# widdowquinn/pyani

Hardware: AMD Instinct MI355X
Metric: genome-pairs/sec (ordered pairs) + wall-clock for the N x N ANIm grid: nucmer --mum + delta-filter -1 + parse_delta equivalent per ordered pair, genomes resident in HBM; vs the CPU path on this box's host cores (higher is better)
Workload: dtype u32 packed DP words (score << 17 | state << 15 | errors), i64 lengths, f64 identity

## Files before the change

### pyani_amd/csrc/pg_anim.hip

```cpp
#include <tuple>
#include "pg_internal.h"
#include "pg_anim_core.h"
#include "pg_nucmer_core.h"
#include "pg_nucmer_diag.h"
#include "pg_anib_core.h"
#include "pg_anim_trace.h"

using namespace pga;

namespace {

constexpr unsigned long long SLOT_EMPTY = ~0ull;
constexpr int FRAG_SEED_MIN = 16;

struct RefDesc {
  const uint32_t* codes;
  const uint32_t* mask;
  int32_t len;
  const int32_t* rec_start;
  int32_t n_rec;
};

struct UnitDesc {
  const uint32_t* codes;
  const uint32_t* mask;
  int32_t len;
  const int32_t* rec_start;
  int32_t n_rec;
  int32_t strand;
  int32_t pair;
  int32_t ref;
};

__device__ __forceinline__ void get16(const uint32_t* __restrict__ codes, const uint32_t* __restrict__ mask, int32_t p,
                                      uint32_t& c, uint32_t& m) {
  const uint32_t cw = p >> 4, cs = 2 * (p & 15);
  const uint64_t lo = (uint64_t)codes[cw] | ((uint64_t)codes[cw + 1] << 32);
  c = (uint32_t)(lo >> cs);
  const uint32_t mw = p >> 5, ms = p & 31;
  const uint64_t ml = (uint64_t)mask[mw] | ((uint64_t)mask[mw + 1] << 32);
  m = (uint32_t)(ml >> ms) & 0xFFFFu;
}

__device__ __forceinline__ void packed_window(const uint32_t* __restrict__ codes, const uint32_t* __restrict__ mask, int32_t len, int64_t p0,
                                              uint64_t& c, uint32_t& ok) {
  c = 0; ok = 0;
  if (p0 >= len || p0 + 32 <= 0) return;
  const int64_t q0 = p0 < 0 ? 0 : p0;
  const int sh = (int)(q0 - p0);
  const int32_t w = (int32_t)(q0 >> 4), lastw = (len - 1) >> 4;
  const uint32_t c0 = codes[w], c1 = codes[w + 1 <= lastw ? w + 1 : lastw], c2 = codes[w + 2 <= lastw ? w + 2 : lastw];
  const int cs = 2 * (int)(q0 & 15);
  uint64_t lo = ((uint64_t)c1 << 32) | c0;
  uint64_t win = cs ? ((lo >> cs) | ((uint64_t)c2 << (64 - cs))) : lo;
  const int32_t mw = (int32_t)(q0 >> 5), lastm = (len - 1) >> 5;
  const uint64_t m = ((uint64_t)mask[mw + 1 <= lastm ? mw + 1 : lastm] << 32) | mask[mw];
  uint32_t okw = (uint32_t)(m >> (q0 & 31));
  const int64_t avail = len - q0;
  if (avail < 32) okw &= (avail <= 0 ? 0u : ((1u << avail) - 1u));
  c = sh ? (win << (2 * sh)) : win;
  ok = sh ? (okw << sh) : okw;
}

#include "pga_seed.inc"
#include "pga_cluster.inc"
#include "pga_postnuc.inc"
#include "pga_finish.inc"
#include "pga_frag.inc"

}

namespace {
struct GenomeIdx {
  uint64_t *ref_list = nullptr, *qry_list = nullptr, *qry_list1 = nullptr;
  uint32_t *ref_goff = nullptr, *qry_goff = nullptr, *qry_goff1 = nullptr;
  uint32_t ref_max = 0;
  uint32_t* word_start = nullptr;
  int32_t* word_pos = nullptr;
};
struct AnimLists { std::vector<GenomeIdx> gidx; };
thread_local PgAlnSink* tls_sink = nullptr;
thread_local int tls_worker = 0;

struct AnimScratch {
  size_t units = 0, pairs = 0, refs = 0, recs = 0, wl = 0, matches = 0;
  uint32_t* list_cnt = nullptr;
  SeedRef* srefs_d = nullptr;
  SeedQry* sqry_d = nullptr;
  SeedSlice* slice_d = nullptr;
  size_t slice_pairs = 0;
  int32_t* recs_d = nullptr;
  RefDesc* refs_d = nullptr;
  UnitDesc* units_d = nullptr;
  uint32_t *mem_count = nullptr, *moff = nullptr, *choff_d = nullptr;
  int32_t *nch = nullptr, *status = nullptr;
  pg_anim_result* out = nullptr;
  Match *mem = nullptr, *cm = nullptr;
  int32_t *iscratch = nullptr, *order = nullptr;
  Chain* chains = nullptr;
  FinishScratch S{};
  uint2* wl_d = nullptr;
  Match* seedbuf = nullptr;
  size_t seed_cap = 0;
  uint32_t* seed_total = nullptr;
  Match* hits_d = nullptr;
  Match* hits_sorted = nullptr;
  uint32_t *hit_count = nullptr, *hoff = nullptr, *hit_cursor = nullptr;
  size_t hit_cap = 0;
  int32_t* mirror_d = nullptr;
  BigUnit* big_d = nullptr;
  uint2* ranges_d = nullptr;
  RangeOut* range_out = nullptr;
  size_t big_cap = 0, range_cap = 0;
  bool lds_attr_set = false;
  pgn::PnAln* pn = nullptr;
  uint8_t* pn_fused = nullptr;
  int32_t* pn_n = nullptr;
  uint32_t* pn_cursor = nullptr;
  uint32_t* pn_gscratch = nullptr;
  uint32_t* pn_wide = nullptr;
  PnForcedReq* pn_reqs = nullptr;
  pgn::PnGap* pn_gaps = nullptr;
  pgn::PnFwd* pn_fwd = nullptr;
  pgn::PnBwd* pn_bwd = nullptr;
  pgn::PnTurn* pn_tlog = nullptr;
  int32_t* pn_born = nullptr;
  uint32_t* pn_porder = nullptr;
  pgn::PnPiece* pn_pieces = nullptr;
  uint32_t* pn_npieces = nullptr;
  size_t pn_piece_cap = 0, pn_npieces_cap = 0;
  uint8_t* tr_arena = nullptr;
  uint32_t* tr_out = nullptr;
  PnTraceJob* tr_jobs = nullptr;
  unsigned long long *tr_off = nullptr, *tr_cursor = nullptr;
  int32_t* tr_cnt = nullptr;
  size_t tr_arena_cap = 0, tr_out_cap = 0, tr_jobs_cap = 0;
  PnGapTask* pn_tasks = nullptr;
  uint32_t* pn_order = nullptr;
  size_t pn_cap = 0, pn_units = 0, pn_waves = 0, pn_req_cap = 0, pn_req_n = 0;
  int32_t* fr_tables = nullptr;
  FragPair* fr_pairs = nullptr;
  uint32_t *fr_slot_pair = nullptr, *fr_off = nullptr, *fr_nrows = nullptr;
  uint64_t* fr_ebase = nullptr;
  FragSeed* fr_entries = nullptr;
  FragRow* fr_rows = nullptr;
  pg_anib_result* fr_out = nullptr;
  uint32_t *fr_list = nullptr, *fr_nlist = nullptr, *fr_wtmp = nullptr;
  WordIdx* fr_widx = nullptr;
  size_t fr_list_cap = 0, fr_widx_cap = 0;
  size_t fr_tables_cap = 0, fr_pairs_cap = 0, fr_slots_cap = 0, fr_off_cap = 0, fr_units_cap = 0, fr_entries_cap = 0;
};

template <typename T>
int regrow(pg_ctx* ctx, T*& p, size_t n) {
  if (p) PG_HIP(ctx, hipFree(p));
  p = nullptr;
  PG_HIP(ctx, hipMalloc(reinterpret_cast<void**>(&p), (n ? n : 1) * sizeof(T)));
  return PG_OK;
}
}

static AnimScratch* anim_scratch(pg_ctx* ctx) {
  void*& slot = tls_worker ? ctx->anim_scratch_w[tls_worker] : ctx->anim_scratch;
  if (!slot) slot = new AnimScratch();
  return static_cast<AnimScratch*>(slot);
}
static AnimLists* anim_lists(pg_ctx* ctx) {
  if (!ctx->anim_lists) ctx->anim_lists = new AnimLists();
  return static_cast<AnimLists*>(ctx->anim_lists);
}
static hipStream_t cur_stream(pg_ctx* ctx) { return tls_worker ? ctx->stream_w[tls_worker] : ctx->stream; }
void pg_anim_set_worker(pg_ctx* ctx, int worker) {
  tls_worker = worker > 0 && worker < pg_ctx::MAX_WORKERS ? worker : 0;
  pg_tls_stream = cur_stream(ctx);
}

void pg_anim_set_sink(PgAlnSink* sink) { tls_sink = sink; }
int pg_anim_counters_read(pg_ctx* ctx, uint64_t* out, int reset) {
  PG_HIP(ctx, hipDeviceSynchronize());
  unsigned long long a[32], b[32], z[32] = {0};
  PG_HIP(ctx, hipMemcpyFromSymbol(a, HIP_SYMBOL(g_pn_stats), sizeof(a)));
  PG_HIP(ctx, hipMemcpyFromSymbol(b, HIP_SYMBOL(g_pn_kstats), sizeof(b)));
  for (int i = 0; i < 32; ++i) { out[i] = a[i]; out[32 + i] = b[i]; }
  if (reset) {
    PG_HIP(ctx, hipMemcpyToSymbol(HIP_SYMBOL(g_pn_stats), z, sizeof(z)));
    PG_HIP(ctx, hipMemcpyToSymbol(HIP_SYMBOL(g_pn_kstats), z, sizeof(z)));
  }
  return PG_OK;
}

void pg_anim_drop_lists(pg_ctx* ctx) {
  std::lock_guard<std::mutex> lk(ctx->anim_mu);
  AnimLists* A = static_cast<AnimLists*>(ctx->anim_lists);
  if (!A) return;
  for (auto& g : A->gidx) {
    void* ptrs[] = {g.ref_list, g.qry_list, g.ref_goff, g.qry_goff, g.qry_list1, g.qry_goff1, g.word_start, g.word_pos};
    for (void* p : ptrs) if (p) (void)hipFree(p);
  }
  A->gidx.clear();
}

static int anim_ensure_lists(pg_ctx* ctx, AnimScratch* A, const std::vector<int32_t>& ref_genomes, const std::vector<int32_t>& qry_genomes,
                             int qstep) {
  std::lock_guard<std::mutex> lk(ctx->anim_mu);
  AnimLists* LS = anim_lists(ctx);
  if (LS->gidx.size() < ctx->genomes.size()) LS->gidx.resize(ctx->genomes.size());
  std::vector<std::pair<uint64_t**, uint32_t**>> mine;
  const int rc_all = [&]() -> int {
  int rc;
  bool built = false;
  if (!A->list_cnt && (rc = regrow(ctx, A->list_cnt, (size_t)2 * SEED_GROUPS))) return rc;
  std::vector<int32_t> fresh_refs;
  for (int role = 0; role < 2; ++role) {
    for (int32_t gid : role ? qry_genomes : ref_genomes) {
      GenomeIdx& X = LS->gidx[gid];
      uint64_t*& qlist = qstep == 1 ? X.qry_list1 : X.qry_list;
      uint32_t*& qgoff = qstep == 1 ? X.qry_goff1 : X.qry_goff;
      if (role ? qlist != nullptr : X.ref_list != nullptr) continue;
      const PgGenome& G = ctx->genomes[gid];
      const int32_t len = (int32_t)G.stream_len;
      const uint32_t n_sub = role ? 2 * SEED_GROUPS : SEED_GROUPS;
      const size_t bound = role ? 2 * ((size_t)len / qstep + 1) : (size_t)len + 1;
      uint64_t*& list = role ? qlist : X.ref_list;
      uint32_t*& goff = role ? qgoff : X.ref_goff;
      mine.emplace_back(&list, &goff);
      if ((rc = regrow(ctx, list, bound))) return rc;
      if ((rc = regrow(ctx, goff, (size_t)n_sub + 2))) return rc;
      const uint32_t* codes = ctx->d_codes + G.arena_start / 16;
      const uint32_t* mask = ctx->d_mask + G.arena_start / 32;
      const int32_t n_idx = role ? len / qstep + 1 : len;
      const dim3 grid((uint32_t)(n_idx + LIST_CHUNK - 1) / LIST_CHUNK, role ? 2 : 1);
      PG_HIP(ctx, hipMemsetAsync(A->list_cnt, 0, (size_t)n_sub * 4, cur_stream(ctx)));
      if (grid.x)
        hipLaunchKernelGGL(anim_list_kernel, grid, dim3(LIST_BLOCK), 0, cur_stream(ctx), codes, mask, len, role, A->list_cnt,
                           (const uint32_t*)nullptr, (uint64_t*)nullptr, 0, qstep);
      hipLaunchKernelGGL(anim_list_scan_kernel, dim3(1), dim3(64), 0, cur_stream(ctx), A->list_cnt, goff, n_sub);
      if (grid.x)
        hipLaunchKernelGGL(anim_list_kernel, grid, dim3(LIST_BLOCK), 0, cur_stream(ctx), codes, mask, len, role, A->list_cnt,
                           (const uint32_t*)goff, list, 1, qstep);
      if (!role) fresh_refs.push_back(gid);
      built = true;
    }
  }
  PG_HIP(ctx, hipGetLastError());
  if (built) PG_HIP(ctx, hipStreamSynchronize(cur_stream(ctx)));
  for (int32_t gid : fresh_refs)
    PG_HIP(ctx, hipMemcpy(&LS->gidx[gid].ref_max, LS->gidx[gid].ref_goff + SEED_GROUPS + 1, 4, hipMemcpyDeviceToHost));
  return PG_OK;
  }();
  if (rc_all != PG_OK) {
    (void)hipStreamSynchronize(cur_stream(ctx));
    for (auto& pr : mine) {
      if (*pr.first) { (void)hipFree(*pr.first); *pr.first = nullptr; }
      if (*pr.second) { (void)hipFree(*pr.second); *pr.second = nullptr; }
    }
  }
  return rc_all;
}

static void anim_free_one(pg_ctx* ctx, void*& slot);
void pg_anim_release_worker_scratch(pg_ctx* ctx) {
  (void)hipStreamSynchronize(ctx->stream);
  for (int w = 1; w < pg_ctx::MAX_WORKERS; ++w) (void)hipStreamSynchronize(ctx->stream_w[w]);
  anim_free_one(ctx, ctx->anim_scratch);
  for (int w = 1; w < pg_ctx::MAX_WORKERS; ++w) anim_free_one(ctx, ctx->anim_scratch_w[w]);
  ctx->anim_scratch_matches_held = 0;
}
void pg_anim_free_scratch(pg_ctx* ctx) {
  pg_anim_drop_lists(ctx);
  delete static_cast<AnimLists*>(ctx->anim_lists);
  ctx->anim_lists = nullptr;
  anim_free_one(ctx, ctx->anim_scratch);
  for (int w = 1; w < pg_ctx::MAX_WORKERS; ++w) anim_free_one(ctx, ctx->anim_scratch_w[w]);
  ctx->anim_scratch_matches_held = 0;
}
static void anim_free_one(pg_ctx* ctx, void*& slot) {
  AnimScratch* A = static_cast<AnimScratch*>(slot);
  if (!A) return;
  void* ptrs[] = {A->mirror_d, A->big_d, A->ranges_d, A->range_out, A->hits_sorted, A->hit_count, A->hoff, A->hit_cursor, A->hits_d, A->slice_d, A->choff_d, A->list_cnt, A->srefs_d, A->sqry_d, A->recs_d, A->refs_d, A->units_d, A->mem_count, A->moff, A->nch, A->status, A->out, A->mem, A->cm,
                  A->iscratch, A->order, A->chains, A->S.alns, A->S.a_rrec,
                  A->S.a_qrec, A->S.idx, A->S.from, A->S.sc, A->wl_d, A->seedbuf, A->seed_total, A->fr_tables, A->fr_pairs,
                  A->fr_slot_pair, A->fr_off, A->fr_nrows, A->fr_ebase, A->fr_entries, A->fr_rows, A->fr_out, A->fr_list, A->fr_nlist, A->fr_wtmp, A->fr_widx,
                  A->pn, A->pn_fused, A->pn_n, A->pn_cursor, A->pn_gscratch, A->pn_reqs, A->pn_wide, A->pn_gaps, A->pn_fwd, A->pn_bwd, A->pn_tlog, A->pn_born, A->pn_porder, A->pn_tasks, A->pn_order, A->pn_pieces, A->pn_npieces, A->tr_arena, A->tr_out, A->tr_jobs, A->tr_off, A->tr_cursor, A->tr_cnt};
  for (void* p : ptrs) if (p) (void)hipFree(p);
  delete A;
  slot = nullptr;
}

static_assert(sizeof(FragRow) == sizeof(pg_anib_row), "FragRow is pg_anib_row");
static int anib_frag_stage(pg_ctx* ctx, AnimScratch* A, const int32_t* qry_ids, uint32_t n_pairs, const std::vector<uint32_t>& cnt,
                           const PgFragArgs& F, const std::vector<int32_t>& ref_list, const std::vector<uint32_t>& ref_of_pair);

static int anim_collect(pg_ctx* ctx, AnimScratch* A, const int32_t* ref_ids, const int32_t* qry_ids, uint32_t n_pairs, const pg_anim_result* res,
                        const std::vector<uint32_t>& choff, PgAlnSink& sink) {
  const uint32_t n_units = 2 * n_pairs;
  int rc;
  std::vector<uint32_t> moff((size_t)n_units + 1);
  PG_HIP(ctx, hipMemcpy(moff.data(), A->moff, moff.size() * 4, hipMemcpyDeviceToHost));
  const size_t total = moff[n_units];
  std::vector<Aln> al(total ? total : 1);
  std::vector<int32_t> rr(total ? total : 1), qr(total ? total : 1);
  if (total) {
    PG_HIP(ctx, hipMemcpy(al.data(), A->S.alns, total * sizeof(Aln), hipMemcpyDeviceToHost));
    PG_HIP(ctx, hipMemcpy(rr.data(), A->S.a_rrec, total * 4, hipMemcpyDeviceToHost));
    PG_HIP(ctx, hipMemcpy(qr.data(), A->S.a_qrec, total * 4, hipMemcpyDeviceToHost));
  }
  const size_t first_aln = sink.alns.size();
  std::vector<size_t> pair_first(n_pairs);
  for (uint32_t p = 0; p < n_pairs; ++p) {
    if (res[p].status == PG_E_CAPACITY) return pg_fail(ctx, PG_E_CAPACITY, "anim: work buffers overflowed for a pair of the batch");
    const PgGenome& G = ctx->genomes[ref_ids[p]];
    const PgGenome& H = ctx->genomes[qry_ids[p]];
    const uint32_t n = (uint32_t)res[p].reserved;
    pair_first[p] = sink.alns.size();
    for (uint32_t i = 0; i < n; ++i) {
      const Aln& a = al[moff[2 * p] + i];
      const int32_t r_ = rr[moff[2 * p] + i], q_ = qr[moff[2 * p] + i], ro = G.rec_start[r_], qo = H.rec_start[q_];
      pg_anim_alignment x;
      x.ref_rec = r_; x.qry_rec = q_;
      x.rs = a.rs - ro + 1; x.re = a.re - ro;
      x.qs = a.strand ? a.qe - qo : a.qs - qo + 1;
      x.qe = a.strand ? a.qs - qo + 1 : a.qe - qo;
      x.errors = a.errors; x.kept = a.keep;
      sink.alns.push_back(x);
    }
    sink.pair_count.push_back(n);
  }
  if (!sink.with_indels) return PG_OK;
  sink.indels.resize(sink.alns.size());
  const size_t n_wl = choff[n_units];
  if (!total || !n_wl) return PG_OK;
  std::vector<pgn::PnAln> pn(total);
  std::vector<int32_t> pn_n(n_units);
  std::vector<uint32_t> npieces(n_units);
  const size_t piece_total = pn_piece_base(total, (uint32_t)n_wl, n_units);
  std::vector<pgn::PnPiece> pieces(piece_total ? piece_total : 1);
  PG_HIP(ctx, hipMemcpy(pn.data(), A->pn, total * sizeof(pgn::PnAln), hipMemcpyDeviceToHost));
  PG_HIP(ctx, hipMemcpy(pn_n.data(), A->pn_n, (size_t)n_units * 4, hipMemcpyDeviceToHost));
  PG_HIP(ctx, hipMemcpy(npieces.data(), A->pn_npieces, (size_t)n_units * 4, hipMemcpyDeviceToHost));
  PG_HIP(ctx, hipMemcpy(pieces.data(), A->pn_pieces, piece_total * sizeof(pgn::PnPiece), hipMemcpyDeviceToHost));
  const size_t req_cap = A->pn_req_n;
  std::vector<PnForcedReq> reqs(req_cap);
  PG_HIP(ctx, hipMemcpy(reqs.data(), A->pn_reqs, req_cap * sizeof(PnForcedReq), hipMemcpyDeviceToHost));
  struct JobRef { uint32_t unit; uint32_t piece; uint64_t bytes; };
  std::vector<PnTraceJob> jobs;
  std::vector<JobRef> refs_;
  for (uint32_t u = 0; u < n_units; ++u) {
    const size_t pb = pn_piece_base(moff[u], choff[u], u);
    if (pn_n[u] < 0 || npieces[u] > pn_piece_cap((size_t)moff[u + 1] - moff[u], choff[u + 1] - choff[u]))
      return pg_fail(ctx, PG_E_CAPACITY, "anim traceback: a unit's piece list overflowed");
    for (uint32_t k = 0; k < npieces[u]; ++k) {
      const pgn::PnPiece& P = pieces[pb + k];
      if (P.kind == pgn::PIECE_MATCH || P.kind == pgn::PIECE_VISIT) continue;
      PnTraceJob J{};
      J.unit = u; J.m_o = P.m_o; J.A0 = P.A0; J.B0 = P.B0; J.A1 = P.A1; J.B1 = P.B1;
      uint64_t cells = P.cells;
      uint32_t wmax = P.wmax;
      if (P.kind == pgn::PIECE_FORCED) {
        J.tA = P.A1; J.tB = P.B1;
        if (P.aux >= req_cap) return pg_fail(ctx, PG_E_INTERNAL, "anim traceback: forced piece without its request");
        J.band_w = reqs[P.aux].w;
        const int32_t N = P.A1 - P.A0 + 1, M_ = P.B1 - P.B0 + 1;
        cells = 0; wmax = 0;
        for (int32_t d = 1; d <= N + M_; ++d) {
          int32_t lo = d - N > 0 ? d - N : 0, hi = d < M_ ? d : M_;
          if (J.band_w >= 0) pgn::forced_band_clip(d, N, M_, J.band_w, lo, hi);
          if (hi >= lo) { cells += (uint64_t)(hi - lo + 1); if ((uint32_t)(hi - lo + 1) > wmax) wmax = (uint32_t)(hi - lo + 1); }
        }
      } else {
        J.tA = P.tA; J.tB = P.tB; J.band_w = -1;
        if (P.cells == 0xFFFFFFFFu) return pg_fail(ctx, PG_E_CAPACITY, "anim traceback: a search outgrew the register engine");
      }
      const int32_t N = J.tA - J.A0 + 1, M_ = J.tB - J.B0 + 1;
      J.cap = wmax + 2; J.dcap = (uint32_t)(N + M_ + 4); J.rle_cap = (uint32_t)(N + M_ + 4); J.bp_cap = cells;
      const uint64_t bytes = (uint64_t)J.cap * 3 * sizeof(pgn::Cell) + (uint64_t)J.dcap * 8 + (uint64_t)J.rle_cap * 4 + ((cells + 15) & ~15ull) + 16;
      jobs.push_back(J);
      refs_.push_back(JobRef{u, k, (bytes + 15) & ~15ull});
    }
  }
  std::vector<uint32_t> order(jobs.size());
  for (uint32_t i = 0; i < order.size(); ++i) order[i] = i;
  std::stable_sort(order.begin(), order.end(), [&](uint32_t a, uint32_t b) { return refs_[a].bytes > refs_[b].bytes; });
  std::vector<std::vector<uint32_t>> rle(jobs.size());
  const uint64_t ARENA = 6ull << 30, OUT_MAX = 192ull << 20;
  if (!A->tr_cursor && (rc = regrow(ctx, A->tr_cursor, 2))) return rc;
  for (size_t b0 = 0; b0 < order.size();) {
    uint64_t bytes = 0, outs = 0;
    size_t b1 = b0;
    while (b1 < order.size() && (b1 == b0 || (bytes + refs_[order[b1]].bytes <= ARENA && outs + jobs[order[b1]].rle_cap <= OUT_MAX))) {
      bytes += refs_[order[b1]].bytes; outs += jobs[order[b1]].rle_cap; ++b1;
    }
    const size_t nb = b1 - b0;
    std::vector<PnTraceJob> hj(nb);
    uint64_t at = 0;
    for (size_t k = 0; k < nb; ++k) { hj[k] = jobs[order[b0 + k]]; hj[k].slab = at; at += refs_[order[b0 + k]].bytes; }
    if (bytes > A->tr_arena_cap) { if ((rc = regrow(ctx, A->tr_arena, (size_t)bytes))) return rc; A->tr_arena_cap = (size_t)bytes; }
    if (outs > A->tr_out_cap) { if ((rc = regrow(ctx, A->tr_out, (size_t)outs))) return rc; A->tr_out_cap = (size_t)outs; }
    if (nb > A->tr_jobs_cap) {
      if ((rc = regrow(ctx, A->tr_jobs, nb))) return rc;
      if ((rc = regrow(ctx, A->tr_off, nb))) return rc;
      if ((rc = regrow(ctx, A->tr_cnt, nb))) return rc;
      A->tr_jobs_cap = nb;
    }
    PG_HIP(ctx, hipMemcpyAsync(A->tr_jobs, hj.data(), nb * sizeof(PnTraceJob), hipMemcpyHostToDevice, cur_stream(ctx)));
    PG_HIP(ctx, hipMemsetAsync(A->tr_cursor, 0, 8, cur_stream(ctx)));
    hipLaunchKernelGGL(anim_trace_kernel, dim3((uint32_t)((nb + 63) / 64)), dim3(64), 0, cur_stream(ctx), A->refs_d, A->units_d, A->tr_jobs, (uint32_t)nb,
                       A->tr_arena, A->tr_out, (unsigned long long)outs, A->tr_cursor, A->tr_off, A->tr_cnt);
    PG_HIP(ctx, hipGetLastError());
    std::vector<unsigned long long> off(nb);
    std::vector<int32_t> cnt(nb);
    unsigned long long used = 0;
    PG_HIP(ctx, hipMemcpyAsync(off.data(), A->tr_off, nb * 8, hipMemcpyDeviceToHost, cur_stream(ctx)));
    PG_HIP(ctx, hipMemcpyAsync(cnt.data(), A->tr_cnt, nb * 4, hipMemcpyDeviceToHost, cur_stream(ctx)));
    PG_HIP(ctx, hipMemcpyAsync(&used, A->tr_cursor, 8, hipMemcpyDeviceToHost, cur_stream(ctx)));
    PG_HIP(ctx, hipStreamSynchronize(cur_stream(ctx)));
    std::vector<uint32_t> out((size_t)used ? (size_t)used : 1);
    if (used) PG_HIP(ctx, hipMemcpy(out.data(), A->tr_out, (size_t)used * 4, hipMemcpyDeviceToHost));
    for (size_t k = 0; k < nb; ++k) {
      if (cnt[k] < 0) return pg_fail(ctx, PG_E_INTERNAL, "anim traceback: a piece did not repeat in the scalar engine");
      rle[order[b0 + k]].assign(out.begin() + (size_t)off[k], out.begin() + (size_t)off[k] + (size_t)cnt[k]);
    }
    b0 = b1;
  }
  size_t job_at = 0;
  for (uint32_t p = 0; p < n_pairs; ++p) {
    const size_t n_rec = (size_t)pn_n[2 * p] + (size_t)pn_n[2 * p + 1];
    if (n_rec != sink.pair_count[sink.pair_count.size() - n_pairs + p]) return pg_fail(ctx, PG_E_INTERNAL, "anim traceback: record counts differ");
    std::vector<std::vector<int64_t>> lists(n_rec);
    std::vector<std::tuple<int32_t, int32_t, int32_t>> key(n_rec);
    for (uint32_t u = 2 * p; u < 2 * p + 2; ++u) {
      const size_t pb = pn_piece_base(moff[u], choff[u], u);
      std::vector<int32_t> job_of(npieces[u], -1);
      for (uint32_t k = 0; k < npieces[u]; ++k)
        if (pieces[pb + k].kind == pgn::PIECE_SEARCH || pieces[pb + k].kind == pgn::PIECE_FORCED) job_of[k] = (int32_t)job_at++;
      std::vector<std::vector<int64_t>> deltas;
      std::vector<int32_t> visit;
      std::string why;
      static const uint32_t none = 0;
      if (!pgt::unit_deltas(pieces.data() + pb, (int32_t)npieces[u], pn.data() + moff[u], pn_n[u],
                            [&](int32_t k, int32_t& c) -> const uint32_t* { const auto& v = rle[(size_t)job_of[k]]; c = (int32_t)v.size(); return v.empty() ? &none : v.data(); },
                            deltas, visit, &why))
        return pg_fail(ctx, PG_E_INTERNAL, "anim traceback: " + why);
      const size_t base = (u & 1) ? (size_t)pn_n[u - 1] : 0;
      for (int32_t i = 0; i < pn_n[u]; ++i) { lists[base + (size_t)i] = std::move(deltas[(size_t)i]); key[base + (size_t)i] = std::make_tuple(visit[(size_t)i], (int32_t)(u & 1), i); }
    }
    std::vector<size_t> perm(n_rec);
    for (size_t i = 0; i < n_rec; ++i) perm[i] = i;
    std::stable_sort(perm.begin(), perm.end(), [&](size_t a, size_t b) { return key[a] < key[b]; });
    std::vector<pg_anim_alignment> recs(n_rec);
    for (size_t i = 0; i < n_rec; ++i) recs[i] = sink.alns[pair_first[p] + perm[i]];
    for (size_t i = 0; i < n_rec; ++i) { sink.alns[pair_first[p] + i] = recs[i]; sink.indels[pair_first[p] + i] = std::move(lists[perm[i]]); }
  }
  (void)first_aln;
  return PG_OK;
}

int pg_anim_run_batch(pg_ctx* ctx, const int32_t* ref_ids, const int32_t* qry_ids, uint32_t n_pairs, int filter_1to1, int maxmatch,
                      uint64_t max_matches, pg_anim_result* out_host, uint32_t* n_done, const PgFragArgs* frag) {
  AnimScratch* A = anim_scratch(ctx);
  int rc;
  (void)hipGetLastError();
  if (frag) {
    uint64_t slots = 0;
    uint32_t fit = 0;
    for (uint32_t p = 0; p < n_pairs; ++p) {
      const PgGenome& Q = ctx->genomes[qry_ids[p]];
      uint64_t nf = 0;
      for (uint32_t r = 0; r < Q.n_rec; ++r) nf += ((uint64_t)(Q.rec_start[r + 1] - 1 - Q.rec_start[r]) + frag->fragsize - 1) / frag->fragsize;
      if (p > 0 && slots + nf > frag->max_slots) break;
      slots += nf;
      fit = p + 1;
    }
    n_pairs = fit;
  }
  uint32_t n_units = 2 * n_pairs;
  const int qstep = frag ? FRAG_QSTEP : SEED_STEP;
  std::vector<int32_t> ref_list;
  std::vector<uint32_t> ref_of_pair(n_pairs);
  for (uint32_t p = 0; p < n_pairs; ++p) {
    if (ref_list.empty() || ref_list.back() != ref_ids[p]) ref_list.push_back(ref_ids[p]);
    ref_of_pair[p] = (uint32_t)ref_list.size() - 1;
  }
  const uint32_t n_refs = (uint32_t)ref_list.size();
  std::vector<RefDesc> refs(n_refs);
  std::vector<int32_t> recs;
  std::vector<uint32_t> ref_rec_off(n_refs), qry_rec_off(n_pairs);
  int32_t max_rlen = 0, max_qlen = 0;
  for (uint32_t r = 0; r < n_refs; ++r) {
    const PgGenome& G = ctx->genomes[ref_list[r]];
    refs[r].codes = ctx->d_codes + G.arena_start / 16;
    refs[r].mask = ctx->d_mask + G.arena_start / 32;
    refs[r].len = (int32_t)G.stream_len;
    refs[r].n_rec = (int32_t)G.n_rec;
    ref_rec_off[r] = (uint32_t)recs.size();
    recs.insert(recs.end(), G.rec_start.begin(), G.rec_start.end());
    if ((int32_t)G.stream_len > max_rlen) max_rlen = (int32_t)G.stream_len;
  }
  for (uint32_t p = 0; p < n_pairs; ++p) {
    const PgGenome& Q = ctx->genomes[qry_ids[p]];
    qry_rec_off[p] = (uint32_t)recs.size();
    recs.insert(recs.end(), Q.rec_start.begin(), Q.rec_start.end());
    if ((int32_t)Q.stream_len > max_qlen) max_qlen = (int32_t)Q.stream_len;
  }
  if (recs.size() > A->recs) { if ((rc = regrow(ctx, A->recs_d, recs.size()))) return rc; A->recs = recs.size(); }
  if (n_refs > A->refs) {
    if ((rc = regrow(ctx, A->refs_d, n_refs))) return rc;
    if ((rc = regrow(ctx, A->srefs_d, n_refs))) return rc;
    A->refs = n_refs;
  }
  if (n_units > A->units) {
    if ((rc = regrow(ctx, A->units_d, n_units))) return rc;
    if ((rc = regrow(ctx, A->mem_count, n_units))) return rc;
    if ((rc = regrow(ctx, A->moff, (size_t)n_units + 1))) return rc;
    if ((rc = regrow(ctx, A->choff_d, (size_t)n_units + 1))) return rc;
    if ((rc = regrow(ctx, A->hit_count, n_units))) return rc;
    if ((rc = regrow(ctx, A->hoff, (size_t)n_units + 1))) return rc;
    if ((rc = regrow(ctx, A->hit_cursor, n_units))) return rc;
    if ((rc = regrow(ctx, A->nch, n_units))) return rc;
    A->units = n_units;
  }
  if (n_pairs > A->pairs) {
    if ((rc = regrow(ctx, A->status, n_pairs))) return rc;
    if ((rc = regrow(ctx, A->sqry_d, n_pairs))) return rc;
    if ((rc = regrow(ctx, A->out, n_pairs))) return rc;
    A->pairs = n_pairs;
  }
  for (uint32_t r = 0; r < n_refs; ++r) refs[r].rec_start = A->recs_d + ref_rec_off[r];
  std::vector<UnitDesc> units(n_units);
  for (uint32_t p = 0; p < n_pairs; ++p) {
    const PgGenome& Q = ctx->genomes[qry_ids[p]];
    for (int s = 0; s < 2; ++s) {
      UnitDesc& U = units[2 * p + s];
      U.codes = ctx->d_codes + Q.arena_start / 16;
      U.mask = ctx->d_mask + Q.arena_start / 32;
      U.len = (int32_t)Q.stream_len;
      U.rec_start = A->recs_d + qry_rec_off[p];
      U.n_rec = (int32_t)Q.n_rec;
      U.strand = s;
      U.pair = (int32_t)p;
      U.ref = (int32_t)ref_of_pair[p];
    }
  }
  PG_HIP(ctx, hipMemcpyAsync(A->recs_d, recs.data(), recs.size() * 4, hipMemcpyHostToDevice, cur_stream(ctx)));
  PG_HIP(ctx, hipMemcpyAsync(A->refs_d, refs.data(), n_refs * sizeof(RefDesc), hipMemcpyHostToDevice, cur_stream(ctx)));
  PG_HIP(ctx, hipMemcpyAsync(A->units_d, units.data(), n_units * sizeof(UnitDesc), hipMemcpyHostToDevice, cur_stream(ctx)));
  std::vector<int32_t> mirror(n_pairs);
  std::vector<uint8_t> seeded(n_pairs);
  std::vector<SeedRef> srefs;
  std::vector<SeedQry> sqry(n_pairs);
  std::vector<GenomeIdx> LSv;
  uint32_t slots = 256, n_srefs = 0;
  if (n_pairs > A->slice_pairs) {
    if ((rc = regrow(ctx, A->slice_d, (size_t)n_pairs * SEED_GROUPS))) return rc;
    if ((rc = regrow(ctx, A->mirror_d, n_pairs))) return rc;
    A->slice_pairs = n_pairs;
  }
  const uint32_t slice_stride = n_pairs;
  const bool use_mirror = !frag && !pg_dev_env("PYANI_ANIM_NO_MIRROR");
  auto prepare = [&](uint32_t limit) -> int {
    std::fill(mirror.begin(), mirror.end(), -1);
    std::fill(seeded.begin(), seeded.end(), (uint8_t)0);
    std::fill(seeded.begin(), seeded.begin() + limit, (uint8_t)1);
    if (use_mirror && limit > 1) {
      std::vector<uint32_t> deg(ctx->genomes.size(), 0);
      for (uint32_t p = 0; p < limit; ++p) ++deg[ref_ids[p]];
      std::vector<uint32_t> idx(limit);
      for (uint32_t p = 0; p < limit; ++p) idx[p] = p;
      auto key = [&](uint32_t p) {
        const uint32_t a = (uint32_t)ref_ids[p], b = (uint32_t)qry_ids[p];
        return std::make_tuple(a < b ? a : b, a < b ? b : a, a < b ? 0 : 1, p);
      };
      std::sort(idx.begin(), idx.end(), [&](uint32_t x, uint32_t y) { return key(x) < key(y); });
      for (uint32_t i = 0; i < limit;) {
        uint32_t j = i;
        while (j < limit && std::get<0>(key(idx[j])) == std::get<0>(key(idx[i])) && std::get<1>(key(idx[j])) == std::get<1>(key(idx[i]))) ++j;
        uint32_t m = i;
        while (m < j && std::get<2>(key(idx[m])) == 0) ++m;
        if (ref_ids[idx[i]] != qry_ids[idx[i]])
          for (uint32_t k = 0; i + k < m && m + k < j; ++k) {
            const uint32_t p = idx[i + k], p2 = idx[m + k];
            const uint32_t a = (uint32_t)ref_ids[p], b = (uint32_t)qry_ids[p];
            const bool first = deg[a] != deg[b] ? deg[a] > deg[b] : ((a < b) != (((a + b) & 1u) != 0));
            if (first) { mirror[p] = (int32_t)p2; seeded[p2] = 0; } else { mirror[p2] = (int32_t)p; seeded[p] = 0; }
          }
        i = j;
      }
    }
    std::vector<int32_t> seed_refs, seed_qrys;
    for (uint32_t p = 0; p < limit; ++p)
      if (seeded[p]) {
        if (seed_refs.empty() || seed_refs.back() != ref_ids[p]) seed_refs.push_back(ref_ids[p]);
        seed_qrys.push_back(qry_ids[p]);
      }
    std::sort(seed_qrys.begin(), seed_qrys.end());
    seed_qrys.erase(std::unique(seed_qrys.begin(), seed_qrys.end()), seed_qrys.end());
    int rc2;
    if ((rc2 = anim_ensure_lists(ctx, A, seed_refs, seed_qrys, qstep))) return rc2;
    {
      std::lock_guard<std::mutex> lk(ctx->anim_mu);
      LSv = anim_lists(ctx)->gidx;
    }
    uint32_t max_group = 1;
    for (int32_t g : seed_refs) if (LSv[g].ref_max > max_group) max_group = LSv[g].ref_max;
    slots = 256;
    while (slots < 2 * max_group) slots <<= 1;
    if (pg_dev_env("PYANI_SEED_SLOTS_MIN")) {
      const uint32_t want = (uint32_t)atoi(pg_dev_env("PYANI_SEED_SLOTS_MIN"));
      while (slots < want && slots < SEED_MAX_SLOTS) slots <<= 1;
    }
    if (slots > SEED_MAX_SLOTS)
      return pg_fail(ctx, PG_E_CAPACITY, "anim seeding: a reference k-mer group does not fit the LDS table (genome too large or too repetitive)");
    srefs.clear();
    for (uint32_t p = 0; p < n_pairs; ++p) {
      sqry[p] = SeedQry{nullptr, nullptr};
      if (p >= limit || !seeded[p]) continue;
      const GenomeIdx& X = LSv[qry_ids[p]];
      sqry[p] = qstep == 1 ? SeedQry{X.qry_list1, X.qry_goff1} : SeedQry{X.qry_list, X.qry_goff};
      if (srefs.empty() || srefs.back().list != LSv[ref_ids[p]].ref_list)
        srefs.push_back(SeedRef{LSv[ref_ids[p]].ref_list, LSv[ref_ids[p]].ref_goff, p, p + 1});
      srefs.back().pair_end = p + 1;
    }
    n_srefs = (uint32_t)srefs.size();
    PG_HIP(ctx, hipMemcpyAsync(A->sqry_d, sqry.data(), n_pairs * sizeof(SeedQry), hipMemcpyHostToDevice, cur_stream(ctx)));
    PG_HIP(ctx, hipMemcpyAsync(A->mirror_d, mirror.data(), n_pairs * sizeof(int32_t), hipMemcpyHostToDevice, cur_stream(ctx)));
    if (n_srefs) PG_HIP(ctx, hipMemcpyAsync(A->srefs_d, srefs.data(), n_srefs * sizeof(SeedRef), hipMemcpyHostToDevice, cur_stream(ctx)));
    hipLaunchKernelGGL(anim_slice_kernel, dim3(n_pairs), dim3(256), 0, cur_stream(ctx), A->sqry_d, slice_stride, A->slice_d);
    return PG_OK;
  };
  if (!A->lds_attr_set) {
    PG_HIP(ctx, hipFuncSetAttribute(reinterpret_cast<const void*>(anim_seed_kernel), hipFuncAttributeMaxDynamicSharedMemorySize,
                                    (int)(SEED_MAX_SLOTS * 8 + SEED_STAGE_BYTES)));
    A->lds_attr_set = true;
  }
  size_t call_bound = 0;
  for (uint32_t p = 0; p < n_pairs && call_bound <= max_matches; ++p)
    call_bound += (size_t)(ctx->genomes[ref_ids[p]].stream_len + ctx->genomes[qry_ids[p]].stream_len) / 4 + 8192;
  const size_t budget = call_bound < max_matches ? call_bound : (size_t)max_matches;
  if (!A->seed_total) {
    if ((rc = regrow(ctx, A->seed_total, 2))) return rc;
  }
  if (budget + 1024 > A->seed_cap) {
    A->seed_cap = budget + 1024;
    if ((rc = regrow(ctx, A->seedbuf, A->seed_cap))) return rc;
  }
  std::vector<uint32_t> cnt(n_units), moff;
  uint32_t total = 0, pairs_fit = 0;
  {
    const size_t want = budget + (size_t)(frag ? 8 * 4096 : 4096) * n_units + 1024;
    if (want > A->hit_cap) {
      if ((rc = regrow(ctx, A->hits_d, want))) return rc;
      if ((rc = regrow(ctx, A->hits_sorted, want))) return rc;
      A->hit_cap = want;
    }
  }
  for (int attempt = 0;; ++attempt) {
    if (attempt == 8) return pg_fail(ctx, PG_E_CAPACITY, "anim seeding: buffers still overflow after repeated splitting");
    uint32_t counts[2] = {0, 0};
    if ((rc = prepare(n_pairs))) return rc;
    PG_HIP(ctx, hipMemsetAsync(A->mem_count, 0, n_units * 4, cur_stream(ctx)));
    PG_HIP(ctx, hipMemsetAsync(A->seed_total, 0, 8, cur_stream(ctx)));
    PG_HIP(ctx, hipMemsetAsync(A->hit_count, 0, n_units * 4, cur_stream(ctx)));
    pg_prof_begin(ctx, PG_K_ANIM_SEED);
    if (n_srefs)
    hipLaunchKernelGGL(anim_seed_kernel, dim3(n_srefs, SEED_GROUPS), dim3(SEED_BLOCK), (size_t)slots * 8 + SEED_STAGE_BYTES, cur_stream(ctx),
                       A->refs_d, A->units_d, A->srefs_d, A->sqry_d, A->slice_d, slice_stride, slots - 1, A->hits_d,
                       (uint32_t)A->hit_cap, A->seed_total + 1, A->hit_count, qstep);
    pg_prof_end(ctx);
    PG_HIP(ctx, hipGetLastError());
    pg_prof_begin(ctx, PG_K_ANIM_HIT);
    hipLaunchKernelGGL(anim_hoff_kernel, dim3(1), dim3(1024), 0, cur_stream(ctx), A->hit_count, n_units, A->hoff, A->hit_cursor);
    hipLaunchKernelGGL(anim_hit_scatter_kernel, dim3((uint32_t)ctx->num_cu * 8u), dim3(256), 0, cur_stream(ctx), A->hits_d, A->seed_total + 1,
                       (uint32_t)A->hit_cap, A->hoff, A->hit_cursor, A->hits_sorted);
    hipLaunchKernelGGL(anim_hit_kernel, dim3(n_units), dim3(256), 0, cur_stream(ctx), A->refs_d, A->units_d, A->hits_sorted, A->hoff,
                       A->seed_total + 1, (uint32_t)A->hit_cap, A->seedbuf, (uint32_t)A->seed_cap, A->seed_total, A->mem_count,
                       frag ? FRAG_SEED_MIN : MIN_MATCH, qstep, use_mirror ? A->mirror_d : (const int32_t*)nullptr);
    pg_prof_end(ctx);
    PG_HIP(ctx, hipMemcpyAsync(cnt.data(), A->mem_count, n_units * 4, hipMemcpyDeviceToHost, cur_stream(ctx)));
    PG_HIP(ctx, hipMemcpyAsync(counts, A->seed_total, 8, hipMemcpyDeviceToHost, cur_stream(ctx)));
    PG_HIP(ctx, hipStreamSynchronize(cur_stream(ctx)));
    total = counts[0];
    if (counts[1] > A->hit_cap) {
      if (n_pairs == 1) {
        A->hit_cap = (size_t)counts[1] + 1024;
        if ((rc = regrow(ctx, A->hits_d, A->hit_cap))) return rc;
        if ((rc = regrow(ctx, A->hits_sorted, A->hit_cap))) return rc;
      } else {
        n_pairs = (n_pairs + 1) / 2;
        n_units = 2 * n_pairs;
      }
      continue;
    }
    uint64_t tot = 0, raw = 0;
    pairs_fit = 0;
    for (uint32_t p = 0; p < n_pairs; ++p) {
      const uint64_t need = (uint64_t)cnt[2 * p] + cnt[2 * p + 1] + 4;
      if (p > 0 && tot + need > max_matches) break;
      tot += need;
      raw += need - 4;
      pairs_fit = p + 1;
    }
    n_pairs = pairs_fit;
    n_units = 2 * n_pairs;
    if (total <= A->seed_cap) break;
    A->seed_cap = (size_t)(raw + raw / 8 + 1024);
    if ((rc = regrow(ctx, A->seedbuf, A->seed_cap))) return rc;
  }
  *n_done = n_pairs;
  moff.assign((size_t)n_units + 1, 0);
  for (uint32_t u = 0; u < n_units; ++u) moff[u + 1] = moff[u] + ((cnt[u] + 2) & ~1u);
  const size_t M = moff[n_units];
  if (M > A->matches) {
    const size_t cap = M + M / 4;
    if ((rc = regrow(ctx, A->mem, cap))) return rc;
    if ((rc = regrow(ctx, A->cm, cap))) return rc;
    if ((rc = regrow(ctx, A->iscratch, cap * 8))) return rc;
    if ((rc = regrow(ctx, A->chains, cap))) return rc;
    if ((rc = regrow(ctx, A->order, cap))) return rc;
    if ((rc = regrow(ctx, A->S.alns, cap))) return rc;
    if ((rc = regrow(ctx, A->S.a_rrec, cap))) return rc;
    if ((rc = regrow(ctx, A->S.a_qrec, cap))) return rc;
    if ((rc = regrow(ctx, A->S.idx, cap))) return rc;
    if ((rc = regrow(ctx, A->S.from, cap))) return rc;
    if ((rc = regrow(ctx, A->S.sc, cap))) return rc;
    __atomic_fetch_add(&ctx->anim_scratch_matches_held, (uint64_t)(cap - A->matches), __ATOMIC_RELAXED);
    A->matches = cap;
  }
  PG_HIP(ctx, hipMemcpyAsync(A->moff, moff.data(), ((size_t)n_units + 1) * 4, hipMemcpyHostToDevice, cur_stream(ctx)));
  PG_HIP(ctx, hipMemsetAsync(A->mem_count, 0, n_units * 4, cur_stream(ctx)));
  PG_HIP(ctx, hipMemsetAsync(A->status, 0, n_pairs * 4, cur_stream(ctx)));
  ClusterOut O{A->moff, A->cm, A->chains, A->nch, A->order, A->status};
  pg_prof_begin(ctx, PG_K_ANIM_HIT);
  if (total)
    hipLaunchKernelGGL(anim_scatter_kernel, dim3((total + 255) / 256), dim3(256), 0, cur_stream(ctx), A->seedbuf, total, A->moff, n_units,
                       A->mem_count, A->mem);
  pg_prof_end(ctx);
  if (frag) {
    PG_HIP(ctx, hipGetLastError());
    return anib_frag_stage(ctx, A, qry_ids, n_pairs, cnt, *frag, ref_list, ref_of_pair);
  }
  const int split_min = pg_dev_env("PYANI_ANIM_SPLIT_MIN") ? atoi(pg_dev_env("PYANI_ANIM_SPLIT_MIN")) : 2048;
  const int range_entries = pg_dev_env("PYANI_ANIM_RANGE_ENTRIES") && atoi(pg_dev_env("PYANI_ANIM_RANGE_ENTRIES")) > 0
                                ? atoi(pg_dev_env("PYANI_ANIM_RANGE_ENTRIES")) : CHAIN_RANGE_ENTRIES;
  std::vector<BigUnit> big;
  std::vector<uint2> ranges;
  if (split_min > 0 && !pg_dev_env("PYANI_ANIM_SCALAR_CLUSTER"))
    for (uint32_t u = 0; u < n_units; ++u)
      if (cnt[u] >= (uint32_t)split_min) {
        uint32_t R = cnt[u] / (uint32_t)range_entries;
        R = R < 1 ? 1 : (R > (uint32_t)CHAIN_RANGES_MAX ? (uint32_t)CHAIN_RANGES_MAX : R);
        for (uint32_t r = 0; r < R; ++r) ranges.push_back(make_uint2((uint32_t)big.size(), r));
        big.push_back(BigUnit{u, (uint32_t)(ranges.size() - R), R, 0});
      }
  if (!big.empty()) {
    if (big.size() > A->big_cap) { if ((rc = regrow(ctx, A->big_d, big.size() + big.size() / 4))) return rc; A->big_cap = big.size() + big.size() / 4; }
    if (ranges.size() > A->range_cap) {
      const size_t c = ranges.size() + ranges.size() / 4;
      if ((rc = regrow(ctx, A->ranges_d, c))) return rc;
      if ((rc = regrow(ctx, A->range_out, c))) return rc;
      A->range_cap = c;
    }
    PG_HIP(ctx, hipMemcpyAsync(A->big_d, big.data(), big.size() * sizeof(BigUnit), hipMemcpyHostToDevice, cur_stream(ctx)));
    PG_HIP(ctx, hipMemcpyAsync(A->ranges_d, ranges.data(), ranges.size() * sizeof(uint2), hipMemcpyHostToDevice, cur_stream(ctx)));
  }
  const int split_arg = big.empty() ? 0x7fffffff : split_min;
  pg_prof_begin(ctx, PG_K_ANIM_CLUSTER);
  if (pg_dev_env("PYANI_ANIM_SCALAR_CLUSTER") && !maxmatch)
    hipLaunchKernelGGL(anim_cluster_kernel, dim3((n_units + 63) / 64), dim3(64), 0, cur_stream(ctx), A->refs_d, A->units_d, n_units,
                       A->mem, A->mem_count, A->iscratch, O);
  else {
    const bool prep = !big.empty() && !pg_dev_env("PYANI_ANIM_WAVE_PREP");
    if (prep)
      hipLaunchKernelGGL(anim_cluster_prep_kernel, dim3((uint32_t)big.size()), dim3(PREP_THREADS), 0, cur_stream(ctx), A->refs_d, A->units_d,
                         A->mem, A->mem_count, A->iscratch, O, maxmatch, A->big_d);
    hipLaunchKernelGGL(anim_cluster_wave_kernel, dim3(n_units), dim3(64), 0, cur_stream(ctx), A->refs_d, A->units_d, A->mem,
                       A->mem_count, A->iscratch, O, prep ? 1 : 0, maxmatch, split_arg);
    if (!big.empty()) {
      hipLaunchKernelGGL(anim_chain_range_kernel, dim3((uint32_t)ranges.size()), dim3(64), 0, cur_stream(ctx), A->units_d, A->mem, A->iscratch,
                         O, A->big_d, A->ranges_d, A->range_out);
      hipLaunchKernelGGL(anim_chain_merge_kernel, dim3((uint32_t)big.size()), dim3(64), 0, cur_stream(ctx), A->refs_d, A->units_d, A->iscratch, O,
                         A->big_d, A->range_out);
    }
  }
  pg_prof_end(ctx);
  std::vector<int32_t> nch(n_units);
  PG_HIP(ctx, hipMemcpyAsync(nch.data(), A->nch, n_units * 4, hipMemcpyDeviceToHost, cur_stream(ctx)));
  PG_HIP(ctx, hipStreamSynchronize(cur_stream(ctx)));
  std::vector<uint32_t> choff((size_t)n_units + 1, 0);
  for (uint32_t u = 0; u < n_units; ++u) choff[u + 1] = choff[u] + (uint32_t)nch[u];
  const size_t n_wl = choff[n_units];
  {
    const size_t Mp = (M + 15) & ~(size_t)15;
    if (Mp > A->pn_cap) {
      if ((rc = regrow(ctx, A->pn, Mp))) return rc;
      if ((rc = regrow(ctx, A->pn_fused, Mp))) return rc;
      if ((rc = regrow(ctx, A->pn_gaps, Mp))) return rc;
      if ((rc = regrow(ctx, A->pn_fwd, Mp))) return rc;
      if ((rc = regrow(ctx, A->pn_bwd, Mp))) return rc;
      if ((rc = regrow(ctx, A->pn_tlog, Mp))) return rc;
      if ((rc = regrow(ctx, A->pn_born, Mp))) return rc;
      if ((rc = regrow(ctx, A->pn_tasks, 4 * Mp))) return rc;
      A->pn_cap = Mp;
    }
    if (n_units > A->pn_units) {
      if ((rc = regrow(ctx, A->pn_n, (size_t)n_units + n_units / 2))) return rc;
      if ((rc = regrow(ctx, A->pn_order, (size_t)n_units + n_units / 2))) return rc;
      if ((rc = regrow(ctx, A->pn_porder, (size_t)n_units + n_units / 2))) return rc;
      A->pn_units = (size_t)n_units + n_units / 2;
    }
    {
      std::vector<uint32_t> uorder(n_units);
      for (uint32_t u = 0; u < n_units; ++u) uorder[u] = u;
      std::stable_sort(uorder.begin(), uorder.end(), [&](uint32_t a, uint32_t b) { return nch[a] > nch[b]; });
      PG_HIP(ctx, hipMemcpyAsync(A->pn_order, uorder.data(), (size_t)n_units * 4, hipMemcpyHostToDevice, cur_stream(ctx)));
      std::vector<uint32_t> porder(n_pairs);
      for (uint32_t p = 0; p < n_pairs; ++p) porder[p] = p;
      std::stable_sort(porder.begin(), porder.end(), [&](uint32_t a, uint32_t b) { return std::max(nch[2 * a], nch[2 * a + 1]) > std::max(nch[2 * b], nch[2 * b + 1]); });
      PG_HIP(ctx, hipMemcpyAsync(A->pn_porder, porder.data(), (size_t)n_pairs * 4, hipMemcpyHostToDevice, cur_stream(ctx)));
      PG_HIP(ctx, hipStreamSynchronize(cur_stream(ctx)));
    }
    if (!A->pn_cursor && (rc = regrow(ctx, A->pn_cursor, 24))) return rc;
    const uint32_t pn_waves = (uint32_t)ctx->num_cu * 12u;
    const uint32_t pn_walk_waves = (uint32_t)ctx->num_cu * 8u;
    const uint32_t pn_waves_pre = (uint32_t)ctx->num_cu * 32u;
    const uint32_t pn_waves_scr = ctx->anim_gap_lanes ? (pn_waves > pn_walk_waves ? pn_waves : pn_walk_waves) : pn_waves_pre;
    if (pn_waves_scr > A->pn_waves) { if ((rc = regrow(ctx, A->pn_gscratch, (size_t)pn_waves_scr * PN_GLOBAL_WORDS))) return rc; A->pn_waves = pn_waves_scr; }
    const bool trace = tls_sink && tls_sink->with_indels;
    const bool bwd_ahead = ctx->anim_bwd_ahead != 0;
    if (trace) {
      const size_t need = pn_piece_base(Mp, (uint32_t)n_wl, n_units) + 16;
      if (need > A->pn_piece_cap) { if ((rc = regrow(ctx, A->pn_pieces, need))) return rc; A->pn_piece_cap = need; }
      if (n_units > A->pn_npieces_cap) { if ((rc = regrow(ctx, A->pn_npieces, (size_t)n_units + 16))) return rc; A->pn_npieces_cap = (size_t)n_units + 16; }
      PG_HIP(ctx, hipMemsetAsync(A->pn_npieces, 0, (size_t)n_units * 4, cur_stream(ctx)));
    }
    const size_t req_cap = Mp + 16;
    A->pn_req_n = req_cap;
    if (req_cap > A->pn_req_cap) { if ((rc = regrow(ctx, A->pn_reqs, req_cap + req_cap / 2))) return rc; if ((rc = regrow(ctx, A->pn_wide, 3 * (req_cap + req_cap / 2)))) return rc; A->pn_req_cap = req_cap + req_cap / 2; }
    PG_HIP(ctx, hipMemsetAsync(A->pn_cursor, 0, 96, cur_stream(ctx)));
    if (n_wl && trace) PG_HIP(ctx, hipMemcpyAsync(A->choff_d, choff.data(), choff.size() * 4, hipMemcpyHostToDevice, cur_stream(ctx)));
    if (n_wl && !trace) {
      if (n_wl > A->wl) { if ((rc = regrow(ctx, A->wl_d, n_wl + n_wl / 2))) return rc; A->wl = n_wl + n_wl / 2; }
      PG_HIP(ctx, hipMemcpyAsync(A->choff_d, choff.data(), choff.size() * 4, hipMemcpyHostToDevice, cur_stream(ctx)));
      hipLaunchKernelGGL(anim_wl_kernel, dim3(n_units), dim3(64), 0, cur_stream(ctx), A->choff_d, A->wl_d);
      pg_prof_begin(ctx, PG_K_ANIM_GAPS);
      const int lane_small = ctx->anim_gap_lanes;
      if (lane_small) {
        hipLaunchKernelGGL(anim_postnuc_gaplist_kernel, dim3((uint32_t)((n_wl + 255) / 256)), dim3(256), 0, cur_stream(ctx), A->units_d, O, A->wl_d,
                           (uint32_t)n_wl, A->pn_tasks, A->pn_cap, A->pn_cursor + 4);
        const dim3 lg((uint32_t)ctx->num_cu * 8u);
        hipLaunchKernelGGL((anim_postnuc_gaplane_kernel<16>), lg, dim3(64), 0, cur_stream(ctx), A->refs_d, A->units_d, O, A->pn_tasks, A->pn_cursor + 4, A->pn_gaps);
        hipLaunchKernelGGL((anim_postnuc_gaplane_kernel<32>), lg, dim3(64), 0, cur_stream(ctx), A->refs_d, A->units_d, O, A->pn_tasks + A->pn_cap, A->pn_cursor + 5, A->pn_gaps);
        hipLaunchKernelGGL((anim_postnuc_gaplane_kernel<PN_SMALL>), lg, dim3(64), 0, cur_stream(ctx), A->refs_d, A->units_d, O, A->pn_tasks + 2 * A->pn_cap, A->pn_cursor + 6, A->pn_gaps);
      }
      if (lane_small)
        hipLaunchKernelGGL(anim_postnuc_gapbig_kernel, dim3(pn_waves_pre), dim3(64), 0, cur_stream(ctx), A->refs_d, A->units_d, O, A->pn_cursor + 3,
                           A->pn_gaps, A->pn_tasks + 3 * A->pn_cap, A->pn_cursor + 11);
      else
        hipLaunchKernelGGL(anim_postnuc_gap_kernel, dim3(pn_waves_pre), dim3(64), 0, cur_stream(ctx), A->refs_d, A->units_d, O, A->wl_d, (uint32_t)n_wl,
                           A->pn_cursor + 3, A->pn_gaps, A->pn_gscratch);
      pg_prof_end(ctx);
      pg_prof_begin(ctx, PG_K_ANIM_FWD);
      hipLaunchKernelGGL(anim_postnuc_fwd_kernel, dim3(pn_waves_pre), dim3(64), 0, cur_stream(ctx), A->refs_d, A->units_d, O, A->wl_d, (uint32_t)n_wl,
                         A->pn_cursor + 8, A->pn_fwd, A->pn_gscratch);
      pg_prof_end(ctx);
      pg_prof_begin(ctx, PG_K_ANIM_BWD);
      if (bwd_ahead) {
        PG_HIP(ctx, hipMemsetAsync(A->pn_bwd, 0, (size_t)M * sizeof(pgn::PnBwd), cur_stream(ctx)));
        hipLaunchKernelGGL(anim_postnuc_rehearse_kernel, dim3(pn_walk_waves < n_units ? pn_walk_waves : n_units), dim3(64), 0, cur_stream(ctx), A->refs_d,
                           A->units_d, n_units, O, A->pn_cursor + 9, A->pn, A->pn_fused, A->pn_gscratch, A->pn_gaps, A->pn_fwd, A->pn_order, A->pn_bwd);
        hipLaunchKernelGGL(anim_postnuc_bwd_kernel, dim3(pn_waves_pre), dim3(64), 0, cur_stream(ctx), A->refs_d, A->units_d, O, A->wl_d, (uint32_t)n_wl,
                           A->pn_cursor + 10, A->pn_bwd, A->pn_gscratch);
      }
      pg_prof_end(ctx);
    }
    pg_prof_begin(ctx, PG_K_ANIM_EXTEND);
    if (n_wl)
      hipLaunchKernelGGL(anim_postnuc_kernel, dim3(pn_walk_waves / 2 < n_pairs ? pn_walk_waves / 2 : n_pairs), dim3(128), 0, cur_stream(ctx), A->refs_d, A->units_d,
                         n_pairs, O, A->pn_cursor, A->pn, A->pn_fused, A->pn_n, A->pn_gscratch, A->pn_reqs, A->pn_cursor + 1, (uint32_t)req_cap,
                         trace ? nullptr : A->pn_gaps, trace ? nullptr : A->pn_fwd, A->pn_porder, trace ? A->pn_pieces : nullptr, A->pn_npieces, A->choff_d,
                         bwd_ahead && !trace ? A->pn_bwd : nullptr, A->pn_tlog, A->pn_born);
    else
      PG_HIP(ctx, hipMemsetAsync(A->pn_n, 0, (size_t)n_units * 4, cur_stream(ctx)));
    pg_prof_end(ctx);
    pg_prof_begin(ctx, PG_K_ANIM_EXTLANE);
    if (n_wl) {
      const uint32_t win_max = (uint32_t)ctx->anim_pn_window_max, group_max = (uint32_t)ctx->anim_pn_group_max;
      hipLaunchKernelGGL(anim_postnuc_forced_kernel, dim3(pn_waves_pre), dim3(64), 0, cur_stream(ctx), A->refs_d, A->units_d, A->pn_reqs,
                         A->pn_cursor + 1, (uint32_t)req_cap, A->pn_cursor + 2, A->pn_n, A->pn_wide, A->pn_cursor + 12, win_max);
      hipLaunchKernelGGL(anim_postnuc_forced_wide_kernel, dim3(pn_waves), dim3(64), 0, cur_stream(ctx), A->refs_d, A->units_d, A->pn_reqs,
                         A->pn_cursor + 1, (uint32_t)req_cap, A->pn_cursor + 13, A->pn_n, A->pn_gscratch, A->pn_wide, A->pn_cursor + 12,
                         A->pn_wide + req_cap, A->pn_cursor + 14, win_max);
      hipLaunchKernelGGL(anim_postnuc_forced_huge_kernel, dim3((uint32_t)ctx->num_cu * 2u), dim3(64 * PN_HUGE_WAVES), 0, cur_stream(ctx), A->refs_d,
                         A->units_d, A->pn_reqs, A->pn_cursor + 15, A->pn_n, A->pn_wide + req_cap, A->pn_cursor + 14, A->pn_wide + 2 * req_cap,
                         A->pn_cursor + 16, group_max);
      hipLaunchKernelGGL(anim_postnuc_forced_strips_kernel, dim3(pn_waves), dim3(64), 0, cur_stream(ctx), A->refs_d, A->units_d, A->pn_reqs,
                         A->pn_cursor + 17, A->pn_n, A->pn_gscratch, A->pn_wide + 2 * req_cap, A->pn_cursor + 16);
    }
    pg_prof_end(ctx);
    if (pg_dev_env("PYANI_PN_STATS")) {
      PG_HIP(ctx, hipStreamSynchronize(cur_stream(ctx)));
      unsigned long long st[32], zero[32] = {0};
      PG_HIP(ctx, hipMemcpyFromSymbol(st, HIP_SYMBOL(g_pn_stats), sizeof(st)));
      PG_HIP(ctx, hipMemcpyToSymbol(HIP_SYMBOL(g_pn_stats), zero, sizeof(zero)));
      fprintf(stderr, "[pn-stats] units %llu clusters %llu | regs: calls %llu steps %llu cells %llu moves %llu overflows %llu | lds: calls %llu steps %llu cells %llu | "
                      "global: calls %llu steps %llu cells %llu\n", st[11], st[12], st[0], st[1], st[2], st[9], st[10], st[3], st[4], st[5], st[6], st[7], st[8]);
      fprintf(stderr, "[pn-stats] searches of the gap + units kernels: %llu calls, %.1f ms inside the engine (summed over waves); shadow tests that asked for the synteny's current alignment: %llu\n", st[22], st[21] / 1e5, st[31]);
      fprintf(stderr, "[pn-stats] forced passes by engine (127 / 255 / 511 cells / strips): %llu %llu %llu %llu passes, %.1f %.1f %.1f %.1f ms summed over waves\n",
              st[27], st[28], st[29], st[30], st[23] / 1e5, st[24] / 1e5, st[25] / 1e5, st[26] / 1e5);
      {
        unsigned long long ks[32], kz[32] = {0};
        PG_HIP(ctx, hipMemcpyFromSymbol(ks, HIP_SYMBOL(g_pn_kstats), sizeof(ks)));
        PG_HIP(ctx, hipMemcpyToSymbol(HIP_SYMBOL(g_pn_kstats), kz, sizeof(kz)));
        const char* kn[8] = {"gaps", "forward", "backward-ahead", "walks", "forced narrow", "forced 512-1024", "forced 2048", "forced group 8192"};
        for (int k = 0; k < 8; ++k)
          fprintf(stderr, "[pn-stats] diagonal engine in %-16s: %llu calls, %llu anti-diagonals, %llu cells\n", kn[k], ks[4 * k], ks[4 * k + 1], ks[4 * k + 2]);
        fprintf(stderr, "[pn-stats] walk kernel scans: shadow test %.1f ms over %llu rows of 64 alignments, reverse-target search %.1f ms in %llu calls (summed over waves)\n",
                ks[3] / 1e5, ks[7], ks[11] / 1e5, ks[15]);
        fprintf(stderr, "[pn-stats] run-ahead results the walk took: forward %llu of %llu computed (%.4f), backward %llu found ready of %llu searches run ahead; %llu searches left to the walk itself\n",
                ks[19], ks[4], ks[4] ? (double)ks[19] / (double)ks[4] : 0.0, ks[23], ks[8], ks[12]);
      }
      for (int k = 13; k <= 17; k += 4)
        fprintf(stderr, "[pn-stats] %s: busy %.1f ms summed over waves, span %.1f ms, longest item %.1f ms (size %llu)\n", k == 13 ? "units" : "forced",
                st[k] / 1e5, st[k + 2] ? (st[k + 2] - ~st[k + 3]) / 1e5 : 0.0, (st[k + 1] >> 20) / 1e5, st[k + 1] & 0xFFFFFull);
    }
  }
  pg_prof_begin(ctx, PG_K_ANIM_FINISH);
  hipLaunchKernelGGL(anim_finish_kernel, dim3(n_pairs), dim3(64), 0, cur_stream(ctx), A->refs_d, A->units_d, n_pairs,
                     O, A->pn, A->pn_n, A->S, filter_1to1, A->out);
  pg_prof_end(ctx);
  PG_HIP(ctx, hipGetLastError());
  PG_HIP(ctx, hipMemcpyAsync(out_host, A->out, n_pairs * sizeof(pg_anim_result), hipMemcpyDeviceToHost, cur_stream(ctx)));
  PG_HIP(ctx, hipStreamSynchronize(cur_stream(ctx)));
  if (tls_sink && (rc = anim_collect(ctx, A, ref_ids, qry_ids, n_pairs, out_host, choff, *tls_sink))) return rc;
  return PG_OK;
}

static int anib_ensure_word_index(pg_ctx* ctx, AnimScratch* A, int32_t gid) {
  int rc;
  std::lock_guard<std::mutex> lk(ctx->anim_mu);
  AnimLists* LS = anim_lists(ctx);
  if (LS->gidx.size() < ctx->genomes.size()) LS->gidx.resize(ctx->genomes.size());
  GenomeIdx& X = LS->gidx[gid];
  if (X.word_start) return PG_OK;
  const PgGenome& G = ctx->genomes[gid];
  const int32_t len = (int32_t)G.stream_len;
  const uint32_t* codes = ctx->d_codes + G.arena_start / 16;
  const uint32_t* mask = ctx->d_mask + G.arena_start / 32;
  uint32_t* start = nullptr;
  int32_t* pos = nullptr;
  if (!A->fr_wtmp && (rc = regrow(ctx, A->fr_wtmp, (size_t)WORD_BUCKETS + 1024 + 16))) return rc;
  if ((rc = regrow(ctx, start, (size_t)WORD_BUCKETS + 1))) return rc;
  if ((rc = regrow(ctx, pos, (size_t)(len > 0 ? len : 1)))) { (void)hipFree(start); return rc; }
  hipStream_t st = cur_stream(ctx);
  const uint32_t grid = (uint32_t)((len + 255) / 256);
  hipError_t e = hipMemsetAsync(start, 0, ((size_t)WORD_BUCKETS + 1) * 4, st);
  if (e == hipSuccess && grid) hipLaunchKernelGGL(anib_word_count_kernel, dim3(grid), dim3(256), 0, st, codes, mask, len, start, pos, 0);
  if (e == hipSuccess) {
    hipLaunchKernelGGL(anib_word_scan1_kernel, dim3(WORD_BUCKETS / 4096u), dim3(1024), 0, st, start, A->fr_wtmp + WORD_BUCKETS);
    hipLaunchKernelGGL(anib_word_scan2_kernel, dim3(1), dim3(1024), 0, st, A->fr_wtmp + WORD_BUCKETS, WORD_BUCKETS / 4096u, start + WORD_BUCKETS);
    hipLaunchKernelGGL(anib_word_scan3_kernel, dim3(WORD_BUCKETS / 1024u), dim3(1024), 0, st, start, A->fr_wtmp + WORD_BUCKETS, A->fr_wtmp);
    if (grid) hipLaunchKernelGGL(anib_word_count_kernel, dim3(grid), dim3(256), 0, st, codes, mask, len, A->fr_wtmp, pos, 1);
    e = hipGetLastError();
  }
  if (e == hipSuccess) e = hipStreamSynchronize(st);
  if (e != hipSuccess) { (void)hipFree(start); (void)hipFree(pos); return pg_fail(ctx, PG_E_HIP, hipGetErrorString(e)); }
  X.word_start = start; X.word_pos = pos;
  return PG_OK;
}

static int anib_frag_stage(pg_ctx* ctx, AnimScratch* A, const int32_t* qry_ids, uint32_t n_pairs, const std::vector<uint32_t>& cnt,
                           const PgFragArgs& F, const std::vector<int32_t>& ref_list, const std::vector<uint32_t>& ref_of_pair) {
  int rc;
  const uint32_t n_units = 2 * n_pairs;
  std::vector<int32_t> tables;
  struct Tab { size_t pos, len, rec0; int32_t n_frags; };
  std::vector<Tab> tab_of(ctx->genomes.size(), Tab{0, 0, 0, -1});
  std::vector<FragPair> fp(n_pairs);
  std::vector<size_t> tab_ref(n_pairs);
  uint64_t slots = 0;
  for (uint32_t p = 0; p < n_pairs; ++p) {
    const int32_t gid = qry_ids[p];
    Tab& T = tab_of[gid];
    if (T.n_frags < 0) {
      const PgGenome& Q = ctx->genomes[gid];
      std::vector<int32_t> pos, len, rec0;
      for (uint32_t r = 0; r < Q.n_rec; ++r) {
        rec0.push_back((int32_t)pos.size());
        const int32_t r0 = Q.rec_start[r], r1 = Q.rec_start[r + 1] - 1;
        for (int32_t f0 = r0; f0 < r1; f0 += F.fragsize) { pos.push_back(f0); len.push_back(r1 - f0 < F.fragsize ? r1 - f0 : F.fragsize); }
      }
      T.n_frags = (int32_t)pos.size();
      T.pos = tables.size(); tables.insert(tables.end(), pos.begin(), pos.end());
      T.len = tables.size(); tables.insert(tables.end(), len.begin(), len.end());
      T.rec0 = tables.size(); tables.insert(tables.end(), rec0.begin(), rec0.end());
    }
    fp[p].n_frags = T.n_frags;
    fp[p].slot0 = (uint32_t)slots;
    slots += (uint64_t)T.n_frags;
  }
  if (slots >= (1ull << 31)) return pg_fail(ctx, PG_E_CAPACITY, "fragment mode: too many (pair, fragment) slots in one launch");
  if (tables.size() + 1 > A->fr_tables_cap) { if ((rc = regrow(ctx, A->fr_tables, tables.size() + 1024))) return rc; A->fr_tables_cap = tables.size() + 1024; }
  for (uint32_t p = 0; p < n_pairs; ++p) {
    const Tab& T = tab_of[qry_ids[p]];
    fp[p].frag_pos = A->fr_tables + T.pos; fp[p].frag_len = A->fr_tables + T.len; fp[p].rec_frag0 = A->fr_tables + T.rec0;
  }
  if (n_pairs > A->fr_pairs_cap) {
    if ((rc = regrow(ctx, A->fr_pairs, n_pairs))) return rc;
    if ((rc = regrow(ctx, A->fr_out, n_pairs))) return rc;
    A->fr_pairs_cap = n_pairs;
  }
  if (n_units > A->fr_units_cap) { if ((rc = regrow(ctx, A->fr_ebase, n_units))) return rc; A->fr_units_cap = n_units; }
  const size_t n_off = 2 * (size_t)slots + 2 * (size_t)n_pairs;
  if (n_off > A->fr_off_cap) { if ((rc = regrow(ctx, A->fr_off, n_off + n_off / 4))) return rc; A->fr_off_cap = n_off + n_off / 4; }
  if (slots > A->fr_slots_cap) {
    const size_t cap = (size_t)slots + (size_t)slots / 4;
    if ((rc = regrow(ctx, A->fr_slot_pair, cap))) return rc;
    if ((rc = regrow(ctx, A->fr_nrows, cap))) return rc;
    if ((rc = regrow(ctx, A->fr_rows, cap * FRAG_ROWS))) return rc;
    A->fr_slots_cap = cap;
  }
  std::vector<uint32_t> slot_pair((size_t)slots);
  for (uint32_t p = 0; p < n_pairs; ++p) std::fill(slot_pair.begin() + fp[p].slot0, slot_pair.begin() + fp[p].slot0 + fp[p].n_frags, p);
  std::vector<uint64_t> ebase(n_units);
  uint64_t n_entries = 0;
  for (uint32_t u = 0; u < n_units; ++u) { ebase[u] = n_entries; n_entries += (uint64_t)cnt[u] + (uint64_t)fp[u / 2].n_frags; }
  if (n_entries > A->fr_entries_cap) { if ((rc = regrow(ctx, A->fr_entries, (size_t)n_entries + (size_t)n_entries / 4))) return rc; A->fr_entries_cap = (size_t)n_entries + (size_t)n_entries / 4; }
  if (!tables.empty()) PG_HIP(ctx, hipMemcpyAsync(A->fr_tables, tables.data(), tables.size() * 4, hipMemcpyHostToDevice, cur_stream(ctx)));
  PG_HIP(ctx, hipMemcpyAsync(A->fr_pairs, fp.data(), n_pairs * sizeof(FragPair), hipMemcpyHostToDevice, cur_stream(ctx)));
  if (slots) PG_HIP(ctx, hipMemcpyAsync(A->fr_slot_pair, slot_pair.data(), (size_t)slots * 4, hipMemcpyHostToDevice, cur_stream(ctx)));
  PG_HIP(ctx, hipMemcpyAsync(A->fr_ebase, ebase.data(), n_units * 8, hipMemcpyHostToDevice, cur_stream(ctx)));
  pg_prof_begin(ctx, PG_K_ANIB_BUCKET);
  hipLaunchKernelGGL(anib_bucket_kernel, dim3(n_units), dim3(256), 0, cur_stream(ctx), A->units_d, A->fr_pairs, A->mem, A->moff, A->mem_count,
                     A->fr_ebase, F.fragsize, A->fr_off, A->fr_entries);
  pg_prof_end(ctx);
  pg_prof_begin(ctx, PG_K_ANIB_FRAG);
  if (slots)
    hipLaunchKernelGGL(anib_frag_kernel, dim3((uint32_t)slots), dim3(64), 0, cur_stream(ctx), A->refs_d, A->units_d, A->fr_pairs, A->fr_slot_pair,
                       A->fr_off, A->fr_entries, A->fr_ebase, A->fr_rows, A->fr_nrows, (const uint32_t*)nullptr, (const WordIdx*)nullptr);
  pg_prof_end(ctx);
  hipLaunchKernelGGL(anib_reduce_pairs_kernel, dim3((n_pairs + 63) / 64), dim3(64), 0, cur_stream(ctx), A->fr_pairs, n_pairs, A->fr_rows, A->fr_nrows,
                     A->fr_out);
  PG_HIP(ctx, hipGetLastError());
  PG_HIP(ctx, hipMemcpyAsync(F.out, A->fr_out, n_pairs * sizeof(pg_anib_result), hipMemcpyDeviceToHost, cur_stream(ctx)));
  PG_HIP(ctx, hipStreamSynchronize(cur_stream(ctx)));
  if (slots && ctx->anib_word_tier) {
    std::vector<WordIdx> widx(ref_list.size(), WordIdx{nullptr, nullptr});
    bool any = false;
    for (uint32_t p = 0; p < n_pairs; ++p) {
      if (!(F.out[p].n_kept > 0 && F.out[p].n_kept < F.out[p].n_frags)) continue;
      const uint32_t r = ref_of_pair[p];
      if (widx[r].start) continue;
      if ((rc = anib_ensure_word_index(ctx, A, ref_list[r]))) return rc;
      const GenomeIdx& X = anim_lists(ctx)->gidx[ref_list[r]];
      widx[r] = WordIdx{X.word_start, X.word_pos};
      any = true;
    }
    if (any) {
      if (widx.size() > A->fr_widx_cap) { if ((rc = regrow(ctx, A->fr_widx, widx.size() + 16))) return rc; A->fr_widx_cap = widx.size() + 16; }
      if ((size_t)slots > A->fr_list_cap) { if ((rc = regrow(ctx, A->fr_list, (size_t)slots + (size_t)slots / 4))) return rc; A->fr_list_cap = (size_t)slots + (size_t)slots / 4; }
      if (!A->fr_nlist && (rc = regrow(ctx, A->fr_nlist, 4))) return rc;
      PG_HIP(ctx, hipMemcpyAsync(A->fr_widx, widx.data(), widx.size() * sizeof(WordIdx), hipMemcpyHostToDevice, cur_stream(ctx)));
      PG_HIP(ctx, hipMemsetAsync(A->fr_nlist, 0, 4, cur_stream(ctx)));
      hipLaunchKernelGGL(anib_failed_kernel, dim3((uint32_t)((slots + 255) / 256)), dim3(256), 0, cur_stream(ctx), A->fr_pairs, A->fr_slot_pair,
                         (uint32_t)slots, A->fr_rows, A->fr_nrows, A->fr_out, A->fr_widx, A->units_d, A->fr_list, A->fr_nlist);
      uint32_t n_list = 0;
      PG_HIP(ctx, hipMemcpyAsync(&n_list, A->fr_nlist, 4, hipMemcpyDeviceToHost, cur_stream(ctx)));
      PG_HIP(ctx, hipStreamSynchronize(cur_stream(ctx)));
      if (n_list) {
        pg_prof_begin(ctx, PG_K_ANIB_FRAG);
        hipLaunchKernelGGL(anib_frag_kernel, dim3(n_list), dim3(64), 0, cur_stream(ctx), A->refs_d, A->units_d, A->fr_pairs, A->fr_slot_pair,
                           A->fr_off, A->fr_entries, A->fr_ebase, A->fr_rows, A->fr_nrows, (const uint32_t*)A->fr_list, (const WordIdx*)A->fr_widx);
        pg_prof_end(ctx);
        hipLaunchKernelGGL(anib_reduce_pairs_kernel, dim3((n_pairs + 63) / 64), dim3(64), 0, cur_stream(ctx), A->fr_pairs, n_pairs, A->fr_rows,
                           A->fr_nrows, A->fr_out);
        PG_HIP(ctx, hipGetLastError());
        PG_HIP(ctx, hipMemcpyAsync(F.out, A->fr_out, n_pairs * sizeof(pg_anib_result), hipMemcpyDeviceToHost, cur_stream(ctx)));
        PG_HIP(ctx, hipStreamSynchronize(cur_stream(ctx)));
      }
    }
  }
  if (F.n_rows_out) {
    const uint32_t nf = (uint32_t)fp[0].n_frags;
    std::vector<uint32_t> nr(nf);
    std::vector<FragRow> rows((size_t)nf * FRAG_ROWS);
    if (nf) {
      PG_HIP(ctx, hipMemcpy(nr.data(), A->fr_nrows + fp[0].slot0, nf * 4, hipMemcpyDeviceToHost));
      PG_HIP(ctx, hipMemcpy(rows.data(), A->fr_rows + (size_t)fp[0].slot0 * FRAG_ROWS, rows.size() * sizeof(FragRow), hipMemcpyDeviceToHost));
    }
    uint32_t n = 0;
    for (uint32_t f = 0; f < nf; ++f)
      for (uint32_t i = 0; i < nr[f]; ++i, ++n)
        if (F.rows_out && n < F.rows_cap) F.rows_out[n] = *reinterpret_cast<const pg_anib_row*>(&rows[(size_t)f * FRAG_ROWS + i]);
    *F.n_rows_out = n;
  }
  return PG_OK;
}

int pg_anim_fetch_alignments(pg_ctx* ctx, int32_t ref_id, int32_t qry_id, uint32_t n, pg_anim_alignment* out) {
  AnimScratch* A = anim_scratch(ctx);
  std::vector<Aln> al(n);
  std::vector<int32_t> rr(n), qr(n);
  if (n) {
    PG_HIP(ctx, hipMemcpy(al.data(), A->S.alns, n * sizeof(Aln), hipMemcpyDeviceToHost));
    PG_HIP(ctx, hipMemcpy(rr.data(), A->S.a_rrec, n * 4, hipMemcpyDeviceToHost));
    PG_HIP(ctx, hipMemcpy(qr.data(), A->S.a_qrec, n * 4, hipMemcpyDeviceToHost));
  }
  const PgGenome& G = ctx->genomes[ref_id];
  const PgGenome& H = ctx->genomes[qry_id];
  for (uint32_t i = 0; i < n; ++i) {
    const Aln& a = al[i];
    const int32_t ro = G.rec_start[rr[i]], qo = H.rec_start[qr[i]];
    pg_anim_alignment x;
    x.ref_rec = rr[i]; x.qry_rec = qr[i];
    x.rs = a.rs - ro + 1; x.re = a.re - ro;
    x.qs = a.strand ? a.qe - qo : a.qs - qo + 1;
    x.qe = a.strand ? a.qs - qo + 1 : a.qe - qo;
    x.errors = a.errors; x.kept = a.keep;
    out[i] = x;
  }
  return PG_OK;
}

int pg_anim_reduce_run(pg_ctx* ctx, uint32_t n_pairs, const uint64_t* offsets, const int32_t* rseq, const int32_t* qseq,
                       const int32_t* rs, const int32_t* re, const int32_t* qs, const int32_t* qe, const int32_t* errors,
                       int apply_filter, pg_anim_result* out) {
  const uint64_t n = offsets[n_pairs];
  std::vector<Aln> h(n);
  for (uint64_t i = 0; i < n; ++i) {
    Aln a;
    a.strand = qs[i] > qe[i];
    a.rs = (rs[i] < re[i] ? rs[i] : re[i]) - 1; a.re = rs[i] < re[i] ? re[i] : rs[i];
    a.qs = (qs[i] < qe[i] ? qs[i] : qe[i]) - 1; a.qe = qs[i] < qe[i] ? qe[i] : qs[i];
    a.errors = errors[i];
    a.keep = apply_filter ? 0 : 3;
    h[i] = a;
  }
  uint64_t* d_off = nullptr; Aln* d_a = nullptr; int32_t *d_rg = nullptr, *d_qg = nullptr, *d_idx = nullptr, *d_from = nullptr;
  double* d_sc = nullptr; pg_anim_result* d_out = nullptr;
  std::vector<void*> to_free;
  auto cleanup = [&]() { for (void* p : to_free) if (p) (void)hipFree(p); };
  int rc;
#define AA(ptr, cnt) do { if ((rc = anim_alloc(ctx, ptr, (cnt)))) { cleanup(); return rc; } to_free.push_back(ptr); } while (0)
  AA(d_off, n_pairs + 1); AA(d_a, n + 1); AA(d_rg, n + 1); AA(d_qg, n + 1); AA(d_idx, n + 1); AA(d_from, n + 1); AA(d_sc, n + 1);
  AA(d_out, n_pairs + 1);
#undef AA
  hipError_t e = hipMemcpyAsync(d_off, offsets, (n_pairs + 1) * 8, hipMemcpyHostToDevice, cur_stream(ctx));
  if (e == hipSuccess && n) e = hipMemcpyAsync(d_a, h.data(), n * sizeof(Aln), hipMemcpyHostToDevice, cur_stream(ctx));
  if (e == hipSuccess && n) e = hipMemcpyAsync(d_rg, rseq, n * 4, hipMemcpyHostToDevice, cur_stream(ctx));
  if (e == hipSuccess && n) e = hipMemcpyAsync(d_qg, qseq, n * 4, hipMemcpyHostToDevice, cur_stream(ctx));
  if (e == hipSuccess) {
    hipLaunchKernelGGL(anim_reduce_kernel, dim3((n_pairs + 63) / 64), dim3(64), 0, cur_stream(ctx), n_pairs, d_off, d_a, d_rg, d_qg,
                       d_idx, d_from, d_sc, apply_filter, d_out);
    e = hipGetLastError();
  }
  if (e == hipSuccess) e = hipMemcpyAsync(out, d_out, n_pairs * sizeof(pg_anim_result), hipMemcpyDeviceToHost, cur_stream(ctx));
  if (e == hipSuccess) e = hipStreamSynchronize(cur_stream(ctx));
  cleanup();
  if (e != hipSuccess) return pg_fail(ctx, PG_E_HIP, std::string("anim reduce: ") + hipGetErrorString(e));
  return PG_OK;
}

namespace {
__global__ __launch_bounds__(64) void anib_reduce_kernel(uint32_t n_pairs, const uint64_t* __restrict__ offsets,
                                                         const uint64_t* __restrict__ foff, const int32_t* __restrict__ frag,
                                                         const int32_t* __restrict__ length, const int32_t* __restrict__ mismatch,
                                                         const int32_t* __restrict__ gaps, const int32_t* __restrict__ qlen,
                                                         const double* __restrict__ pident, int64_t* first_row,
                                                         int64_t* __restrict__ aln_out, int64_t* __restrict__ err_out,
                                                         double* __restrict__ pid_out) {
  const uint32_t p = blockIdx.x * blockDim.x + threadIdx.x;
  if (p >= n_pairs) return;
  int64_t* first = first_row + foff[p];
  const uint64_t nf = foff[p + 1] - foff[p];
  for (uint64_t f = 0; f < nf; ++f) first[f] = -1;
  for (uint64_t i = offsets[p]; i < offsets[p + 1]; ++i) {
    const int32_t alnlen = length[i] - gaps[i], alnids = alnlen - mismatch[i];
    const double cov = (double)alnlen / (double)qlen[i], pid = (double)alnids / (double)qlen[i];
    if (cov > 0.7 && pid > 0.3 && (uint64_t)frag[i] < nf && first[frag[i]] < 0) first[frag[i]] = (int64_t)i;
  }
  int64_t aln = 0, err = 0, cnt = 0;
  double sum = 0.0;
  for (uint64_t f = 0; f < nf; ++f) {
    const int64_t i = first[f];
    if (i < 0) continue;
    aln += length[i] - gaps[i];
    err += (int64_t)mismatch[i] + gaps[i];
    sum = sum + pident[i];
    ++cnt;
  }
  aln_out[p] = aln;
  err_out[p] = err;
  pid_out[p] = cnt ? sum / (double)cnt : 0.0;
}
}

int pg_anib_reduce_run(pg_ctx* ctx, uint32_t n_pairs, const uint64_t* offsets, const uint32_t* n_frags, const int32_t* frag,
                       const int32_t* length, const int32_t* mismatch, const int32_t* gaps, const int32_t* qlen,
                       const double* pident, int64_t* aln_out, int64_t* err_out, double* pid_out) {
  const uint64_t n = offsets[n_pairs];
  std::vector<uint64_t> foff(n_pairs + 1, 0);
  for (uint32_t p = 0; p < n_pairs; ++p) foff[p + 1] = foff[p] + n_frags[p];
  std::vector<void*> to_free;
  auto cleanup = [&]() { for (void* q : to_free) if (q) (void)hipFree(q); };
  uint64_t *d_off = nullptr, *d_foff = nullptr;
  int32_t *d_frag = nullptr, *d_len = nullptr, *d_mm = nullptr, *d_gap = nullptr, *d_ql = nullptr;
  double *d_pid = nullptr, *d_pout = nullptr;
  int64_t *d_first = nullptr, *d_aln = nullptr, *d_err = nullptr;
  int rc;
#define AA(ptr, cnt) do { if ((rc = anim_alloc(ctx, ptr, (cnt)))) { cleanup(); return rc; } to_free.push_back(ptr); } while (0)
  AA(d_off, n_pairs + 1); AA(d_foff, n_pairs + 1); AA(d_frag, n + 1); AA(d_len, n + 1); AA(d_mm, n + 1); AA(d_gap, n + 1);
  AA(d_ql, n + 1); AA(d_pid, n + 1); AA(d_first, foff[n_pairs] + 1); AA(d_aln, n_pairs); AA(d_err, n_pairs); AA(d_pout, n_pairs);
#undef AA
  hipError_t e = hipMemcpyAsync(d_off, offsets, (n_pairs + 1) * 8, hipMemcpyHostToDevice, cur_stream(ctx));
  if (e == hipSuccess) e = hipMemcpyAsync(d_foff, foff.data(), (n_pairs + 1) * 8, hipMemcpyHostToDevice, cur_stream(ctx));
  const struct { void* d; const void* h; size_t b; } cp[] = {{d_frag, frag, n * 4}, {d_len, length, n * 4}, {d_mm, mismatch, n * 4},
                                                           {d_gap, gaps, n * 4}, {d_ql, qlen, n * 4}, {d_pid, pident, n * 8}};
  for (const auto& c : cp)
    if (e == hipSuccess && c.b) e = hipMemcpyAsync(c.d, c.h, c.b, hipMemcpyHostToDevice, cur_stream(ctx));
  if (e == hipSuccess) {
    hipLaunchKernelGGL(anib_reduce_kernel, dim3((n_pairs + 63) / 64), dim3(64), 0, cur_stream(ctx), n_pairs, d_off, d_foff, d_frag, d_len,
                       d_mm, d_gap, d_ql, d_pid, d_first, d_aln, d_err, d_pout);
    e = hipGetLastError();
  }
  if (e == hipSuccess) e = hipMemcpyAsync(aln_out, d_aln, n_pairs * 8, hipMemcpyDeviceToHost, cur_stream(ctx));
  if (e == hipSuccess) e = hipMemcpyAsync(err_out, d_err, n_pairs * 8, hipMemcpyDeviceToHost, cur_stream(ctx));
  if (e == hipSuccess) e = hipMemcpyAsync(pid_out, d_pout, n_pairs * 8, hipMemcpyDeviceToHost, cur_stream(ctx));
  if (e == hipSuccess) e = hipStreamSynchronize(cur_stream(ctx));
  cleanup();
  if (e != hipSuccess) return pg_fail(ctx, PG_E_HIP, std::string("anib reduce: ") + hipGetErrorString(e));
  return PG_OK;
}
```

### pyani_amd/csrc/pga_seed.inc

```

constexpr int SEED_K = 16, SEED_STEP = 5;
static_assert(SEED_K + SEED_STEP - 1 == MIN_MATCH, "sampling must not miss a minimal-length match");

__device__ __forceinline__ bool seed_kmer(const uint32_t* __restrict__ codes, const uint32_t* __restrict__ mask, int32_t len,
                                          int32_t strand, int32_t q, uint32_t& k) {
  uint32_t c, m;
  if (strand == 0) {
    get16(codes, mask, q, c, m);
    k = c;
  } else {
    get16(codes, mask, len - SEED_K - q, c, m);
    uint32_t x = __brev(c);
    x = ((x & 0xAAAAAAAAu) >> 1) | ((x & 0x55555555u) << 1);
    k = ~x;
  }
  return m == 0xFFFFu;
}

constexpr int SEED_GROUP_BITS = 11, SEED_GROUPS = 1 << SEED_GROUP_BITS;
constexpr uint32_t SEED_MAX_SLOTS = 16384;
__device__ __forceinline__ uint32_t seed_hash(uint32_t k) { return k * 0x9E3779B1u; }
__device__ __forceinline__ uint32_t seed_group(uint32_t h) { return h >> (32 - SEED_GROUP_BITS); }

constexpr uint64_t SEED_KEY_SHIFT = 43;
constexpr int LIST_BLOCK = 1024, LIST_CHUNK = 16384;
__global__ __launch_bounds__(LIST_BLOCK) void anim_list_kernel(const uint32_t* __restrict__ codes, const uint32_t* __restrict__ mask,
                                                               int32_t len, int role, uint32_t* __restrict__ cnt,
                                                               const uint32_t* __restrict__ goff, uint64_t* __restrict__ list, int pass,
                                                               int step) {
  __shared__ uint32_t s_cnt[2 * SEED_GROUPS];
  const int32_t strand = role ? (int32_t)blockIdx.y : 0;
  const uint32_t n_sub = role ? 2 * SEED_GROUPS : SEED_GROUPS;
  const int32_t idx0 = blockIdx.x * LIST_CHUNK;
  for (uint32_t i = threadIdx.x; i < n_sub; i += LIST_BLOCK) s_cnt[i] = 0;
  __syncthreads();
  auto kmer_of = [&](int32_t idx, uint32_t& h, int32_t& p) -> bool {
    p = role ? idx * step : idx;
    if (p + SEED_K > len) return false;
    uint32_t k;
    if (!seed_kmer(codes, mask, len, strand, p, k)) return false;
    h = seed_hash(k);
    return true;
  };
  auto sub_of = [&](uint32_t h) { const uint32_t g = seed_group(h); return role ? 2 * g + (uint32_t)strand : g; };
  for (int32_t t = threadIdx.x; t < LIST_CHUNK; t += LIST_BLOCK) {
    uint32_t h; int32_t p;
    if (kmer_of(idx0 + t, h, p)) atomicAdd(&s_cnt[sub_of(h)], 1u);
  }
  __syncthreads();
  for (uint32_t i = threadIdx.x; i < n_sub; i += LIST_BLOCK) {
    const uint32_t c = s_cnt[i];
    uint32_t base = 0;
    if (c) base = atomicAdd(&cnt[i], c);
    s_cnt[i] = pass ? goff[i] + base : 0;
  }
  if (!pass) return;
  __syncthreads();
  const StrandView V{SeqView{codes, mask, len}, strand};
  for (int32_t t = threadIdx.x; t < LIST_CHUNK; t += LIST_BLOCK) {
    uint32_t h; int32_t p;
    if (!kmer_of(idx0 + t, h, p)) continue;
    const uint32_t at = atomicAdd(&s_cnt[sub_of(h)], 1u);
    uint64_t left = 0, flag = 1;
    for (int j = 1; j <= SEED_STEP; ++j) {
      if (!V.clean(p - j)) { flag = 0; left = 0; break; }
      left |= (uint64_t)V.base(p - j) << (2 * (j - 1));
    }
    list[at] = ((uint64_t)(h & 0x1FFFFFu) << SEED_KEY_SHIFT) | (left << 33) | (flag << 32) | (uint32_t)p;
  }
}

__global__ __launch_bounds__(64) void anim_list_scan_kernel(uint32_t* __restrict__ cnt, uint32_t* __restrict__ goff, uint32_t n) {
  const uint32_t lane = threadIdx.x;
  uint32_t run = 0, mx = 0;
  for (uint32_t base = 0; base < n; base += 64) {
    const uint32_t c = cnt[base + lane];
    cnt[base + lane] = 0;
    uint32_t incl = c;
#pragma unroll
    for (int o = 1; o < 64; o <<= 1) { const uint32_t t = __shfl_up(incl, o, 64); if ((int)lane >= o) incl += t; }
    goff[base + lane] = run + incl - c;
    run += __shfl(incl, 63, 64);
    mx = c > mx ? c : mx;
  }
#pragma unroll
  for (int o = 32; o > 0; o >>= 1) { const uint32_t t = __shfl_xor(mx, o, 64); mx = t > mx ? t : mx; }
  if (lane == 0) { goff[n] = run; goff[n + 1] = mx; }
}

struct SeedRef {
  const uint64_t* list;
  const uint32_t* goff;
  uint32_t pair_begin, pair_end;
};
struct SeedQry {
  const uint64_t* list;
  const uint32_t* goff;
};
struct SeedSlice { uint32_t begin, n0, n1; };
__global__ __launch_bounds__(256) void anim_slice_kernel(const SeedQry* __restrict__ sqry, uint32_t n_pairs, SeedSlice* __restrict__ slice) {
  const uint32_t p = blockIdx.x;
  const uint32_t* goff = sqry[p].goff;
  for (uint32_t g = threadIdx.x; g < SEED_GROUPS; g += 256) {
    if (!goff) { slice[(size_t)g * n_pairs + p] = SeedSlice{0, 0, 0}; continue; }
    const uint32_t o0 = goff[2 * g], o1 = goff[2 * g + 1], o2 = goff[2 * g + 2];
    slice[(size_t)g * n_pairs + p] = SeedSlice{o0, o1 - o0, o2 - o1};
  }
}

__device__ __forceinline__ bool seed_hit(const RefDesc& R, const SeqView& RV, const UnitDesc& U0, const StrandView& QV, int strand,
                                         int32_t r, int32_t q, int32_t left, int32_t min_match, int32_t step, Match& out) {
  if (left < 0) {
    left = 0;
    while (left < step && RV.clean(r - 1 - left) && QV.clean(q - 1 - left) && RV.base(r - 1 - left) == QV.base(q - 1 - left)) ++left;
  }
  if (left >= step) return false;
  int32_t L = SEED_K;
  int n = 16;
  while (n == 16 && r + L + 16 <= R.len && q + L + 16 <= U0.len) {
    uint32_t rc_, rm_, qc_, qm_;
    get16(R.codes, R.mask, r + L, rc_, rm_);
    uint32_t fc, fm;
    get16(U0.codes, U0.mask, strand == 0 ? q + L : U0.len - 16 - (q + L), fc, fm);
    uint32_t rv = __brev(fc);
    rv = ((rv & 0xAAAAAAAAu) >> 1) | ((rv & 0x55555555u) << 1);
    qc_ = strand == 0 ? fc : ~rv;
    qm_ = strand == 0 ? fm : __brev(fm) >> 16;
    const uint32_t x = rc_ ^ qc_;
    const uint32_t diff = (x | (x >> 1)) & 0x55555555u;
    const uint32_t bad = ~(rm_ & qm_) & 0xFFFFu;
    const int nd = diff ? (__ffs(diff) - 1) >> 1 : 16;
    const int nb = bad ? __ffs(bad) - 1 : 16;
    n = nd < nb ? nd : nb;
    L += n;
  }
  if (n == 16)
    while (RV.clean(r + L) && QV.clean(q + L) && RV.base(r + L) == QV.base(q + L)) ++L;
  if (left + L < min_match) return false;
  out = Match{r - left, q - left, left + L, 0};
  return true;
}

constexpr int SEED_BLOCK = 1024, SEED_UNROLL = 4;
constexpr uint32_t SEED_STAGE = 48;
constexpr size_t SEED_STAGE_BYTES = (SEED_BLOCK / 64) * (SEED_STAGE * sizeof(Match) + 4);
__global__ __launch_bounds__(SEED_BLOCK) void anim_seed_kernel(const RefDesc* __restrict__ refs, const UnitDesc* __restrict__ units,
                                                               const SeedRef* __restrict__ srefs, const SeedQry* __restrict__ sqry,
                                                               const SeedSlice* __restrict__ slice, uint32_t n_pairs,
                                                               uint32_t slot_mask, Match* __restrict__ buf, uint32_t cap,
                                                               uint32_t* __restrict__ total, uint32_t* __restrict__ hit_count, int32_t step) {
  extern __shared__ __attribute__((aligned(16))) unsigned long long tab[];
  Match* stage = reinterpret_cast<Match*>(tab + slot_mask + 1);
  uint32_t* stage_n = reinterpret_cast<uint32_t*>(stage + (SEED_BLOCK / 64) * SEED_STAGE);
  const uint32_t g = blockIdx.y;
  const SeedRef SR = srefs[blockIdx.x];
  const uint32_t tid = threadIdx.x, lane = tid & 63u, wave = tid >> 6;
  for (uint32_t i = tid; i <= slot_mask; i += SEED_BLOCK) tab[i] = SLOT_EMPTY;
  if (tid < SEED_BLOCK / 64) stage_n[tid] = 0;
  __syncthreads();
  for (uint32_t e = SR.goff[g] + tid; e < SR.goff[g + 1]; e += SEED_BLOCK) {
    const unsigned long long v = SR.list[e];
    uint32_t slot = (uint32_t)(v >> (SEED_KEY_SHIFT + 5)) & slot_mask;
    while (atomicCAS(&tab[slot], SLOT_EMPTY, v) != SLOT_EMPTY) slot = (slot + 1) & slot_mask;
  }
  __syncthreads();
  const uint32_t n_mine_all = SR.pair_end - SR.pair_begin;
  const uint32_t per_wave = (n_mine_all + SEED_BLOCK / 64 - 1) / (SEED_BLOCK / 64);
  const uint32_t my_begin = SR.pair_begin + wave * per_wave;
  const uint32_t my_end = my_begin + per_wave < SR.pair_end ? my_begin + per_wave : SR.pair_end;
  const SeedSlice* __restrict__ row = slice + (size_t)g * n_pairs;
  for (uint32_t chunk = my_begin; chunk < my_end; chunk += 64) {
    SeedSlice mine{0, 0, 0};
    const uint64_t* mylist = nullptr;
    if (chunk + lane < my_end) { mine = row[chunk + lane]; mylist = sqry[chunk + lane].list; }
    const uint32_t in_chunk = my_end - chunk < 64 ? my_end - chunk : 64;
    struct Blk { uint32_t j, strand, e0, e_end; const uint64_t* list; bool valid; };
    auto slice_of = [&](uint32_t j, uint32_t strand, Blk& o) {
      const uint32_t begin = (uint32_t)__builtin_amdgcn_readlane((int)mine.begin, j);
      const uint32_t n0 = (uint32_t)__builtin_amdgcn_readlane((int)mine.n0, j), n1 = (uint32_t)__builtin_amdgcn_readlane((int)mine.n1, j);
      o.j = j; o.strand = strand;
      o.e0 = strand ? begin + n0 : begin;
      o.e_end = o.e0 + (strand ? n1 : n0);
      o.list = reinterpret_cast<const uint64_t*>(
          ((unsigned long long)(uint32_t)__builtin_amdgcn_readlane((int)((unsigned long long)mylist >> 32), j) << 32) |
          (unsigned long long)(uint32_t)__builtin_amdgcn_readlane((int)(unsigned long long)mylist, j));
    };
    auto first_from = [&](uint32_t j, uint32_t strand) {
      Blk o{0, 0, 0, 0, nullptr, false};
      for (; j < in_chunk; ++j, strand = 0)
        for (; strand < 2; ++strand) {
          slice_of(j, strand, o);
          if (o.e0 < o.e_end) { o.valid = true; return o; }
        }
      return o;
    };
    auto next_of = [&](const Blk& c) {
      if (c.e0 + 64 * SEED_UNROLL < c.e_end) { Blk o = c; o.e0 += 64 * SEED_UNROLL; return o; }
      return c.strand == 0 ? first_from(c.j, 1) : first_from(c.j + 1, 0);
    };
    auto load = [&](const Blk& c, unsigned long long (&qv)[SEED_UNROLL]) {
#pragma unroll
      for (int t = 0; t < SEED_UNROLL; ++t) {
        const uint32_t e = c.e0 + 64 * t + lane;
        qv[t] = e < c.e_end ? __builtin_nontemporal_load(&c.list[e]) : SLOT_EMPTY;
      }
    };
    auto process = [&](const Blk& c, const unsigned long long (&qv)[SEED_UNROLL], bool last) {
      const uint32_t unit = 2 * (chunk + c.j) + c.strand;
#pragma unroll
      for (int t = 0; t < SEED_UNROLL; ++t) {
        if (qv[t] == SLOT_EMPTY) continue;
        const uint32_t key = (uint32_t)(qv[t] >> SEED_KEY_SHIFT);
        const uint32_t qctx = (uint32_t)(qv[t] >> 32) & 0x7FFu;
        const int32_t q = (int32_t)(uint32_t)qv[t];
        uint32_t slot_b = ((key >> 5) & slot_mask) << 3;
        const uint32_t byte_mask = (slot_mask << 3) | 7u;
        const char* const tab_b = reinterpret_cast<const char*>(tab);
        const uint32_t qhi = (uint32_t)(qv[t] >> 32);
        unsigned long long v = *reinterpret_cast<const unsigned long long*>(tab_b + slot_b);
        while ((uint32_t)v != 0xFFFFFFFFu) {
          if ((((uint32_t)(v >> 32) ^ qhi) >> (SEED_KEY_SHIFT - 32)) == 0u) {
            int32_t left = -1;
            bool report = true;
            const uint32_t rctx = (uint32_t)(v >> 32) & 0x7FFu;
            if (rctx & qctx & 1u) {
              const uint32_t x = (rctx ^ qctx) >> 1;
              const uint32_t diff = (x | (x >> 1)) & 0x155u;
              left = diff ? (__ffs(diff) - 1) >> 1 : SEED_STEP;
              report = left < step;
            }
            if (report) {
              const Match m{(int32_t)(uint32_t)v, q, left, (int32_t)unit};
              const uint32_t at = atomicAdd(&stage_n[wave], 1u);
              if (at < SEED_STAGE) {
                stage[wave * SEED_STAGE + at] = m;
              } else {
                const uint32_t ga = atomicAdd(total, 1u);
                atomicAdd(&hit_count[unit], 1u);
                if (ga < cap) buf[ga] = m;
              }
            }
          }
          slot_b = (slot_b + 8u) & byte_mask;
          v = *reinterpret_cast<const unsigned long long*>(tab_b + slot_b);
        }
      }
      __builtin_amdgcn_wave_barrier();
      uint32_t n_st = stage_n[wave];
      if (n_st > SEED_STAGE) n_st = SEED_STAGE;
      if (n_st >= SEED_STAGE / 2 || (n_st && last)) {
        static_assert(SEED_STAGE <= 64, "one staged hit per lane at flush time");
        uint32_t base = 0;
        if (lane == 0) {
          base = atomicAdd(total, n_st);
          stage_n[wave] = 0;
        }
        base = __shfl(base, 0);
        Match m{0, 0, 0, -1};
        if (lane < n_st) m = stage[wave * SEED_STAGE + lane];
        const int32_t prev_unit = __shfl_up(m.strand, 1, 64);
        const bool start = lane < n_st && (lane == 0 || prev_unit != m.strand);
        const uint64_t starts = __ballot(start);
        if (start) {
          const uint64_t later = starts >> 1 >> lane;
          const uint32_t run = later ? (uint32_t)__ffsll((unsigned long long)later) : n_st - lane;
          atomicAdd(&hit_count[(uint32_t)m.strand], run);
        }
        if (lane < n_st && base + lane < cap) buf[base + lane] = m;
        __builtin_amdgcn_wave_barrier();
      }
    };
    unsigned long long qa[SEED_UNROLL], qb[SEED_UNROLL];
    Blk A = first_from(0, 0);
    if (A.valid) load(A, qa);
    while (A.valid) {
      Blk B = next_of(A);
      if (B.valid) load(B, qb);
      process(A, qa, !B.valid && chunk + 64 >= my_end);
      if (!B.valid) break;
      A = next_of(B);
      if (A.valid) load(A, qa);
      process(B, qb, !A.valid && chunk + 64 >= my_end);
    }
  }
}

__global__ __launch_bounds__(1024) void anim_hoff_kernel(const uint32_t* __restrict__ cnt, uint32_t n, uint32_t* __restrict__ hoff,
                                                         uint32_t* __restrict__ cursor) {
  __shared__ uint32_t s_part[1024];
  const uint32_t tid = threadIdx.x;
  const uint32_t per = (n + 1023) / 1024, lo = tid * per, hi = lo + per < n ? lo + per : n;
  uint32_t sum = 0;
  for (uint32_t i = lo; i < hi; ++i) sum += cnt[i];
  s_part[tid] = sum;
  __syncthreads();
  if (tid == 0) { uint32_t run = 0; for (int i = 0; i < 1024; ++i) { const uint32_t t = s_part[i]; s_part[i] = run; run += t; } hoff[n] = run; }
  __syncthreads();
  uint32_t run = s_part[tid];
  for (uint32_t i = lo; i < hi; ++i) { hoff[i] = run; run += cnt[i]; cursor[i] = 0; }
}

__global__ __launch_bounds__(256) void anim_hit_scatter_kernel(const Match* __restrict__ buf, const uint32_t* __restrict__ n_hits, uint32_t cap,
                                                               const uint32_t* __restrict__ hoff, uint32_t* __restrict__ cursor,
                                                               Match* __restrict__ out) {
  const uint32_t n = *n_hits < cap ? *n_hits : cap;
  const uint32_t lane = threadIdx.x & 63u;
  for (uint32_t base = blockIdx.x * blockDim.x; base < n; base += gridDim.x * blockDim.x) {
    const uint32_t i = base + threadIdx.x;
    Match m{0, 0, 0, 0};
    if (i < n) m = buf[i];
    const uint32_t u = (uint32_t)m.strand;
    bool todo = i < n;
    while (true) {
      const uint64_t rest = __ballot(todo);
      if (!rest) break;
      const int leader = __ffsll((unsigned long long)rest) - 1;
      const uint32_t lu = __shfl(u, leader);
      const uint64_t same = __ballot(todo && u == lu);
      uint32_t at = 0;
      if ((int)lane == leader) at = atomicAdd(&cursor[lu], (uint32_t)__popcll(same));
      at = __shfl(at, leader);
      if (todo && u == lu) {
        out[(size_t)hoff[u] + at + (uint32_t)__popcll(same & ((1ull << lane) - 1ull))] = m;
        todo = false;
      }
    }
  }
}

__global__ __launch_bounds__(256) void anim_hit_kernel(const RefDesc* __restrict__ refs, const UnitDesc* __restrict__ units,
                                                       const Match* __restrict__ hits, const uint32_t* __restrict__ hoff,
                                                       const uint32_t* __restrict__ n_hits, uint32_t hit_cap,
                                                       Match* __restrict__ buf, uint32_t cap, uint32_t* __restrict__ total,
                                                       uint32_t* __restrict__ unit_count, int32_t min_match, int32_t step,
                                                       const int32_t* __restrict__ mirror) {
  const uint32_t unit = blockIdx.x;
  const uint32_t h0 = hoff[unit], h1 = hoff[unit + 1];
  if (h0 == h1 || *n_hits > hit_cap) return;
  const uint32_t lane = threadIdx.x & 63u;
  const UnitDesc U0 = units[unit];
  const RefDesc R = refs[U0.ref];
  const SeqView RV{R.codes, R.mask, R.len};
  const StrandView QV{SeqView{U0.codes, U0.mask, U0.len}, U0.strand};
  const int32_t mp = mirror ? mirror[U0.pair] : -1;
  const uint32_t unit2 = mp >= 0 ? 2u * (uint32_t)mp + (uint32_t)U0.strand : 0u;
  for (uint32_t base = h0; base < h1; base += blockDim.x) {
    const uint32_t i = base + threadIdx.x;
    Match m{0, 0, 0, (int32_t)unit};
    bool have = false;
    if (i < h1) {
      const Match h = hits[i];
      have = seed_hit(R, RV, U0, QV, U0.strand, h.r, h.q, h.len, min_match, step, m);
    }
    const uint64_t got = __ballot(have);
    if (got) {
      uint32_t at = 0;
      const uint32_t c = (uint32_t)__popcll(got);
      if (lane == 0) {
        at = atomicAdd(total, mp >= 0 ? 2 * c : c);
        atomicAdd(&unit_count[unit], c);
        if (mp >= 0) atomicAdd(&unit_count[unit2], c);
      }
      at = __shfl(at, 0);
      if (have) {
        at += (uint32_t)__popcll(got & ((1ull << lane) - 1ull));
        m.strand = (int32_t)unit;
        if (at < cap) buf[at] = m;
        if (mp >= 0 && at + c < cap)
          buf[at + c] = U0.strand == 0 ? Match{m.q, m.r, m.len, (int32_t)unit2}
                                       : Match{U0.len - m.q - m.len, R.len - m.r - m.len, m.len, (int32_t)unit2};
      }
    }
  }
}

__global__ __launch_bounds__(256) void anim_scatter_kernel(const Match* __restrict__ buf, uint32_t n, const uint32_t* __restrict__ moff,
                                                           uint32_t n_units, uint32_t* __restrict__ cursor, Match* __restrict__ mem) {
  const uint32_t i = blockIdx.x * blockDim.x + threadIdx.x;
  const uint32_t lane = threadIdx.x & 63u;
  Match m{0, 0, 0, -1};
  if (i < n) m = buf[i];
  const uint32_t u = (uint32_t)m.strand;
  bool todo = i < n && u < n_units;
  while (true) {
    const uint64_t rest = __ballot(todo);
    if (!rest) break;
    const int leader = __ffsll((unsigned long long)rest) - 1;
    const uint32_t lu = __shfl(u, leader);
    const uint64_t same = __ballot(todo && u == lu);
    uint32_t base = 0;
    if ((int)lane == leader) base = atomicAdd(&cursor[lu], (uint32_t)__popcll(same));
    base = __shfl(base, leader);
    if (todo && u == lu) {
      m.strand = (int32_t)(u & 1u);
      mem[(size_t)moff[u] + base + (uint32_t)__popcll(same & ((1ull << lane) - 1ull))] = m;
      todo = false;
    }
  }
}
```

Before: 65290.

## Batch multiple references per seed block with finer hash groups and shared LDS table

Seeding now packs several reference genomes into one workgroup's LDS hash table, using finer k-mer groups so each group fits, and streams the union of their queries against it. A host-built pair table maps (slot, query) codes back to pair units. This amortises the table build and query-list reads across many pairs instead of one reference per block. The list-scan kernel is rewritten as a 1024-thread templated scan to handle the larger group count. It adds host-side block planning, extra device tables and more complex hit-code decoding. The old per-pair path remains behind an environment variable.

Result: faster. 68800 (median of 6 runs) (+5.4%).

```diff
diff --git a/pyani_amd/csrc/pg_anim.hip b/pyani_amd/csrc/pg_anim.hip
--- a/pyani_amd/csrc/pg_anim.hip
+++ b/pyani_amd/csrc/pg_anim.hip
@@ -1,4 +1,5 @@
 #include <tuple>
+#include <unordered_map>
 #include "pg_internal.h"
 #include "pg_anim_core.h"
 #include "pg_nucmer_core.h"
@@ -75,6 +76,7 @@
   uint64_t *ref_list = nullptr, *qry_list = nullptr, *qry_list1 = nullptr;
   uint32_t *ref_goff = nullptr, *qry_goff = nullptr, *qry_goff1 = nullptr;
   uint32_t ref_max = 0;
+  uint32_t ref_max_fine = 0;
   uint32_t* word_start = nullptr;
   int32_t* word_pos = nullptr;
 };
@@ -89,6 +91,11 @@
   SeedQry* sqry_d = nullptr;
   SeedSlice* slice_d = nullptr;
   size_t slice_pairs = 0;
+  SeedBlk* sblk_d = nullptr;
+  SeedSlot* sslot_d = nullptr;
+  SeedQry* sbq_d = nullptr;
+  int32_t* spt_d = nullptr;
+  size_t sblk_cap = 0, sslot_cap = 0, sbq_cap = 0, spt_cap = 0;
   int32_t* recs_d = nullptr;
   RefDesc* refs_d = nullptr;
   UnitDesc* units_d = nullptr;
@@ -209,7 +216,11 @@
   const int rc_all = [&]() -> int {
   int rc;
   bool built = false;
-  if (!A->list_cnt && (rc = regrow(ctx, A->list_cnt, (size_t)2 * SEED_GROUPS))) return rc;
+  if (!A->list_cnt) {
+    if ((rc = regrow(ctx, A->list_cnt, (size_t)2 * SEED_GROUPS))) return rc;
+    PG_HIP(ctx, hipFuncSetAttribute(reinterpret_cast<const void*>(anim_list_kernel), hipFuncAttributeMaxDynamicSharedMemorySize,
+                                    (int)(2 * SEED_GROUPS * 4)));
+  }
   std::vector<int32_t> fresh_refs;
   for (int role = 0; role < 2; ++role) {
     for (int32_t gid : role ? qry_genomes : ref_genomes) {
@@ -225,18 +236,21 @@
       uint32_t*& goff = role ? qgoff : X.ref_goff;
       mine.emplace_back(&list, &goff);
       if ((rc = regrow(ctx, list, bound))) return rc;
-      if ((rc = regrow(ctx, goff, (size_t)n_sub + 2))) return rc;
+      if ((rc = regrow(ctx, goff, (size_t)n_sub + 3))) return rc;
       const uint32_t* codes = ctx->d_codes + G.arena_start / 16;
       const uint32_t* mask = ctx->d_mask + G.arena_start / 32;
       const int32_t n_idx = role ? len / qstep + 1 : len;
       const dim3 grid((uint32_t)(n_idx + LIST_CHUNK - 1) / LIST_CHUNK, role ? 2 : 1);
       PG_HIP(ctx, hipMemsetAsync(A->list_cnt, 0, (size_t)n_sub * 4, cur_stream(ctx)));
       if (grid.x)
-        hipLaunchKernelGGL(anim_list_kernel, grid, dim3(LIST_BLOCK), 0, cur_stream(ctx), codes, mask, len, role, A->list_cnt,
+        hipLaunchKernelGGL(anim_list_kernel, grid, dim3(LIST_BLOCK), (size_t)n_sub * 4, cur_stream(ctx), codes, mask, len, role, A->list_cnt,
                            (const uint32_t*)nullptr, (uint64_t*)nullptr, 0, qstep);
-      hipLaunchKernelGGL(anim_list_scan_kernel, dim3(1), dim3(64), 0, cur_stream(ctx), A->list_cnt, goff, n_sub);
+      if (role)
+        hipLaunchKernelGGL(anim_list_scan_kernel<2 * SEED_GROUPS / LIST_SCAN_BLOCK>, dim3(1), dim3(LIST_SCAN_BLOCK), 0, cur_stream(ctx), A->list_cnt, goff);
+      else
+        hipLaunchKernelGGL(anim_list_scan_kernel<SEED_GROUPS / LIST_SCAN_BLOCK>, dim3(1), dim3(LIST_SCAN_BLOCK), 0, cur_stream(ctx), A->list_cnt, goff);
       if (grid.x)
-        hipLaunchKernelGGL(anim_list_kernel, grid, dim3(LIST_BLOCK), 0, cur_stream(ctx), codes, mask, len, role, A->list_cnt,
+        hipLaunchKernelGGL(anim_list_kernel, grid, dim3(LIST_BLOCK), (size_t)n_sub * 4, cur_stream(ctx), codes, mask, len, role, A->list_cnt,
                            (const uint32_t*)goff, list, 1, qstep);
       if (!role) fresh_refs.push_back(gid);
       built = true;
@@ -244,8 +258,12 @@
   }
   PG_HIP(ctx, hipGetLastError());
   if (built) PG_HIP(ctx, hipStreamSynchronize(cur_stream(ctx)));
-  for (int32_t gid : fresh_refs)
-    PG_HIP(ctx, hipMemcpy(&LS->gidx[gid].ref_max, LS->gidx[gid].ref_goff + SEED_GROUPS + 1, 4, hipMemcpyDeviceToHost));
+  for (int32_t gid : fresh_refs) {
+    uint32_t mx[2];
+    PG_HIP(ctx, hipMemcpy(mx, LS->gidx[gid].ref_goff + SEED_GROUPS + 1, 8, hipMemcpyDeviceToHost));
+    LS->gidx[gid].ref_max_fine = mx[0];
+    LS->gidx[gid].ref_max = mx[1];
+  }
   return PG_OK;
   }();
   if (rc_all != PG_OK) {
@@ -277,7 +295,7 @@
 static void anim_free_one(pg_ctx* ctx, void*& slot) {
   AnimScratch* A = static_cast<AnimScratch*>(slot);
   if (!A) return;
-  void* ptrs[] = {A->mirror_d, A->big_d, A->ranges_d, A->range_out, A->hits_sorted, A->hit_count, A->hoff, A->hit_cursor, A->hits_d, A->slice_d, A->choff_d, A->list_cnt, A->srefs_d, A->sqry_d, A->recs_d, A->refs_d, A->units_d, A->mem_count, A->moff, A->nch, A->status, A->out, A->mem, A->cm,
+  void* ptrs[] = {A->mirror_d, A->big_d, A->ranges_d, A->range_out, A->hits_sorted, A->hit_count, A->hoff, A->hit_cursor, A->hits_d, A->slice_d, A->sblk_d, A->sslot_d, A->sbq_d, A->spt_d, A->choff_d, A->list_cnt, A->srefs_d, A->sqry_d, A->recs_d, A->refs_d, A->units_d, A->mem_count, A->moff, A->nch, A->status, A->out, A->mem, A->cm,
                   A->iscratch, A->order, A->chains, A->S.alns, A->S.a_rrec,
                   A->S.a_qrec, A->S.idx, A->S.from, A->S.sc, A->wl_d, A->seedbuf, A->seed_total, A->fr_tables, A->fr_pairs,
                   A->fr_slot_pair, A->fr_off, A->fr_nrows, A->fr_ebase, A->fr_entries, A->fr_rows, A->fr_out, A->fr_list, A->fr_nlist, A->fr_wtmp, A->fr_widx,
@@ -523,6 +541,7 @@
     if ((rc = regrow(ctx, A->status, n_pairs))) return rc;
     if ((rc = regrow(ctx, A->sqry_d, n_pairs))) return rc;
     if ((rc = regrow(ctx, A->out, n_pairs))) return rc;
+    if ((rc = regrow(ctx, A->mirror_d, n_pairs))) return rc;
     A->pairs = n_pairs;
   }
   for (uint32_t r = 0; r < n_refs; ++r) refs[r].rec_start = A->recs_d + ref_rec_off[r];
@@ -549,14 +568,19 @@
   std::vector<SeedRef> srefs;
   std::vector<SeedQry> sqry(n_pairs);
   std::vector<GenomeIdx> LSv;
-  uint32_t slots = 256, n_srefs = 0;
-  if (n_pairs > A->slice_pairs) {
-    if ((rc = regrow(ctx, A->slice_d, (size_t)n_pairs * SEED_GROUPS))) return rc;
-    if ((rc = regrow(ctx, A->mirror_d, n_pairs))) return rc;
-    A->slice_pairs = n_pairs;
-  }
+  uint32_t slots = 256, n_srefs = 0, n_blks = 0, slot_shift = 0;
   const uint32_t slice_stride = n_pairs;
   const bool use_mirror = !frag && !pg_dev_env("PYANI_ANIM_NO_MIRROR");
+  const bool use_blocks = !frag && !(pg_dev_env("PYANI_SEED_PER_PAIR") && atoi(pg_dev_env("PYANI_SEED_PER_PAIR")) == 1);
+  uint32_t blk_slots = SEED_MAX_SLOTS;
+  if (pg_dev_env("PYANI_SEED_BLOCK_SLOTS")) {
+    const int want = atoi(pg_dev_env("PYANI_SEED_BLOCK_SLOTS"));
+    blk_slots = want >= 512 && want <= (int)SEED_MAX_SLOTS ? (uint32_t)want : SEED_MAX_SLOTS;
+  }
+  std::vector<SeedBlk> blks;
+  std::vector<SeedSlot> bslots;
+  std::vector<SeedQry> bqry;
+  std::vector<int32_t> bpair;
   auto prepare = [&](uint32_t limit) -> int {
     std::fill(mirror.begin(), mirror.end(), -1);
     std::fill(seeded.begin(), seeded.end(), (uint8_t)0);
@@ -600,6 +624,74 @@
       std::lock_guard<std::mutex> lk(ctx->anim_mu);
       LSv = anim_lists(ctx)->gidx;
     }
+    if (use_blocks) {
+      std::vector<int32_t> slot_ref;
+      std::vector<std::vector<uint32_t>> slot_pairs;
+      std::unordered_map<int32_t, uint32_t> occ;
+      uint32_t run_first = 0;
+      int32_t run_ref = -1;
+      for (uint32_t p = 0; p < limit; ++p) {
+        if (!seeded[p]) continue;
+        if (ref_ids[p] != run_ref) { run_ref = ref_ids[p]; run_first = (uint32_t)slot_ref.size(); occ.clear(); }
+        const uint32_t k = occ[qry_ids[p]]++;
+        if (run_first + k == slot_ref.size()) { slot_ref.push_back(run_ref); slot_pairs.emplace_back(); }
+        slot_pairs[run_first + k].push_back(p);
+      }
+      blks.clear(); bslots.clear(); bqry.clear(); bpair.clear();
+      uint32_t max_sum = 1;
+      for (uint32_t s0 = 0; s0 < slot_ref.size();) {
+        uint32_t s1 = s0, sum = 0;
+        while (s1 < slot_ref.size() && s1 - s0 < (uint32_t)SEED_BLOCK_SLOTS) {
+          const uint32_t w = LSv[slot_ref[s1]].ref_max_fine;
+          if (s1 > s0 && 2 * (sum + w) > blk_slots) break;
+          sum += w;
+          ++s1;
+        }
+        max_sum = sum > max_sum ? sum : max_sum;
+        std::vector<int32_t> qs;
+        for (uint32_t t = s0; t < s1; ++t) {
+          const PgGenome& G = ctx->genomes[slot_ref[t]];
+          if (G.stream_len >= SEED_TAB_POS_MASK)
+            return pg_fail(ctx, PG_E_CAPACITY, "anim seeding: a reference position does not fit the block table's 30 bits");
+          bslots.push_back(SeedSlot{LSv[slot_ref[t]].ref_list, LSv[slot_ref[t]].ref_goff});
+          for (uint32_t p : slot_pairs[t]) qs.push_back(qry_ids[p]);
+        }
+        std::sort(qs.begin(), qs.end());
+        qs.erase(std::unique(qs.begin(), qs.end()), qs.end());
+        if (qs.size() >= (1u << 25)) return pg_fail(ctx, PG_E_CAPACITY, "anim seeding: more than 2^25 queries in a block");
+        const SeedBlk Bk{s0, s1, (uint32_t)bqry.size(), (uint32_t)(bqry.size() + qs.size()), (uint32_t)bpair.size()};
+        for (int32_t qg : qs) bqry.push_back(SeedQry{LSv[qg].qry_list, LSv[qg].qry_goff});
+        bpair.resize(bpair.size() + (size_t)(s1 - s0) * qs.size(), -1);
+        for (uint32_t t = s0; t < s1; ++t)
+          for (uint32_t p : slot_pairs[t]) {
+            const size_t qi = (size_t)(std::lower_bound(qs.begin(), qs.end(), qry_ids[p]) - qs.begin());
+            bpair[Bk.pair_tab + (size_t)(t - s0) * qs.size() + qi] = (int32_t)p;
+          }
+        blks.push_back(Bk);
+        s0 = s1;
+      }
+      if (bpair.size() > (size_t)0x7FFFFFFF) return pg_fail(ctx, PG_E_CAPACITY, "anim seeding: block pair tables too large");
+      slots = 256;
+      while (slots < 2 * max_sum) slots <<= 1;
+      if (slots > SEED_MAX_SLOTS)
+        return pg_fail(ctx, PG_E_CAPACITY, "anim seeding: a reference k-mer group does not fit the LDS table (genome too large or too repetitive)");
+      slot_shift = 0;
+      while ((slots << slot_shift) < (1u << (32 - SEED_GROUP_BITS))) ++slot_shift;
+      n_blks = (uint32_t)blks.size();
+      int rc3;
+      if (n_blks > A->sblk_cap) { if ((rc3 = regrow(ctx, A->sblk_d, n_blks))) return rc3; A->sblk_cap = n_blks; }
+      if (bslots.size() > A->sslot_cap) { if ((rc3 = regrow(ctx, A->sslot_d, bslots.size()))) return rc3; A->sslot_cap = bslots.size(); }
+      if (bqry.size() > A->sbq_cap) { if ((rc3 = regrow(ctx, A->sbq_d, bqry.size()))) return rc3; A->sbq_cap = bqry.size(); }
+      if (bpair.size() > A->spt_cap) { if ((rc3 = regrow(ctx, A->spt_d, bpair.size()))) return rc3; A->spt_cap = bpair.size(); }
+      if (n_blks) {
+        PG_HIP(ctx, hipMemcpyAsync(A->sblk_d, blks.data(), n_blks * sizeof(SeedBlk), hipMemcpyHostToDevice, cur_stream(ctx)));
+        PG_HIP(ctx, hipMemcpyAsync(A->sslot_d, bslots.data(), bslots.size() * sizeof(SeedSlot), hipMemcpyHostToDevice, cur_stream(ctx)));
+        PG_HIP(ctx, hipMemcpyAsync(A->sbq_d, bqry.data(), bqry.size() * sizeof(SeedQry), hipMemcpyHostToDevice, cur_stream(ctx)));
+        PG_HIP(ctx, hipMemcpyAsync(A->spt_d, bpair.data(), bpair.size() * sizeof(int32_t), hipMemcpyHostToDevice, cur_stream(ctx)));
+      }
+      PG_HIP(ctx, hipMemcpyAsync(A->mirror_d, mirror.data(), n_pairs * sizeof(int32_t), hipMemcpyHostToDevice, cur_stream(ctx)));
+      return PG_OK;
+    }
     uint32_t max_group = 1;
     for (int32_t g : seed_refs) if (LSv[g].ref_max > max_group) max_group = LSv[g].ref_max;
     slots = 256;
@@ -610,6 +702,10 @@
     }
     if (slots > SEED_MAX_SLOTS)
       return pg_fail(ctx, PG_E_CAPACITY, "anim seeding: a reference k-mer group does not fit the LDS table (genome too large or too repetitive)");
+    if (slice_stride > A->slice_pairs) {
+      if ((rc2 = regrow(ctx, A->slice_d, (size_t)slice_stride * SEED_CGROUPS))) return rc2;
+      A->slice_pairs = slice_stride;
+    }
     srefs.clear();
     for (uint32_t p = 0; p < n_pairs; ++p) {
       sqry[p] = SeedQry{nullptr, nullptr};
@@ -630,6 +726,8 @@
   if (!A->lds_attr_set) {
     PG_HIP(ctx, hipFuncSetAttribute(reinterpret_cast<const void*>(anim_seed_kernel), hipFuncAttributeMaxDynamicSharedMemorySize,
                                     (int)(SEED_MAX_SLOTS * 8 + SEED_STAGE_BYTES)));
+    PG_HIP(ctx, hipFuncSetAttribute(reinterpret_cast<const void*>(anim_seed_pair_kernel), hipFuncAttributeMaxDynamicSharedMemorySize,
+                                    (int)(SEED_MAX_SLOTS * 8 + SEED_STAGE_BYTES)));
     A->lds_attr_set = true;
   }
   size_t call_bound = 0;
@@ -661,10 +759,14 @@
     PG_HIP(ctx, hipMemsetAsync(A->seed_total, 0, 8, cur_stream(ctx)));
     PG_HIP(ctx, hipMemsetAsync(A->hit_count, 0, n_units * 4, cur_stream(ctx)));
     pg_prof_begin(ctx, PG_K_ANIM_SEED);
-    if (n_srefs)
-    hipLaunchKernelGGL(anim_seed_kernel, dim3(n_srefs, SEED_GROUPS), dim3(SEED_BLOCK), (size_t)slots * 8 + SEED_STAGE_BYTES, cur_stream(ctx),
-                       A->refs_d, A->units_d, A->srefs_d, A->sqry_d, A->slice_d, slice_stride, slots - 1, A->hits_d,
-                       (uint32_t)A->hit_cap, A->seed_total + 1, A->hit_count, qstep);
+    if (use_blocks && n_blks)
+      hipLaunchKernelGGL(anim_seed_kernel, dim3(n_blks, SEED_GROUPS), dim3(SEED_BLOCK), (size_t)slots * 8 + SEED_STAGE_BYTES, cur_stream(ctx),
+                         A->sblk_d, A->sslot_d, A->sbq_d, A->spt_d, slots - 1, slot_shift, A->hits_d, (uint32_t)A->hit_cap,
+                         A->seed_total + 1, A->hit_count, qstep);
+    else if (!use_blocks && n_srefs)
+      hipLaunchKernelGGL(anim_seed_pair_kernel, dim3(n_srefs, SEED_CGROUPS), dim3(SEED_BLOCK), (size_t)slots * 8 + SEED_STAGE_BYTES, cur_stream(ctx),
+                         A->srefs_d, A->sqry_d, A->slice_d, slice_stride, slots - 1, A->hits_d, (uint32_t)A->hit_cap, A->seed_total + 1,
+                         A->hit_count, qstep);
     pg_prof_end(ctx);
     PG_HIP(ctx, hipGetLastError());
     pg_prof_begin(ctx, PG_K_ANIM_HIT);
diff --git a/pyani_amd/csrc/pga_seed.inc b/pyani_amd/csrc/pga_seed.inc
--- a/pyani_amd/csrc/pga_seed.inc
+++ b/pyani_amd/csrc/pga_seed.inc
@@ -17,18 +17,22 @@
   return m == 0xFFFFu;
 }
 
-constexpr int SEED_GROUP_BITS = 11, SEED_GROUPS = 1 << SEED_GROUP_BITS;
+constexpr int SEED_GROUP_BITS = 14, SEED_GROUPS = 1 << SEED_GROUP_BITS;
+constexpr int SEED_CGROUP_BITS = 11, SEED_CGROUPS = 1 << SEED_CGROUP_BITS, SEED_SUB = SEED_GROUPS / SEED_CGROUPS;
 constexpr uint32_t SEED_MAX_SLOTS = 16384;
 __device__ __forceinline__ uint32_t seed_hash(uint32_t k) { return k * 0x9E3779B1u; }
 __device__ __forceinline__ uint32_t seed_group(uint32_t h) { return h >> (32 - SEED_GROUP_BITS); }
 
 constexpr uint64_t SEED_KEY_SHIFT = 43;
 constexpr int LIST_BLOCK = 1024, LIST_CHUNK = 16384;
+__device__ __forceinline__ uint32_t seed_sub(uint32_t g, int role, uint32_t strand) {
+  return role ? ((2u * (g >> 3) + strand) << 3) + (g & 7u) : g;
+}
 __global__ __launch_bounds__(LIST_BLOCK) void anim_list_kernel(const uint32_t* __restrict__ codes, const uint32_t* __restrict__ mask,
                                                                int32_t len, int role, uint32_t* __restrict__ cnt,
                                                                const uint32_t* __restrict__ goff, uint64_t* __restrict__ list, int pass,
                                                                int step) {
-  __shared__ uint32_t s_cnt[2 * SEED_GROUPS];
+  extern __shared__ uint32_t s_cnt[];
   const int32_t strand = role ? (int32_t)blockIdx.y : 0;
   const uint32_t n_sub = role ? 2 * SEED_GROUPS : SEED_GROUPS;
   const int32_t idx0 = blockIdx.x * LIST_CHUNK;
@@ -42,7 +46,7 @@
     h = seed_hash(k);
     return true;
   };
-  auto sub_of = [&](uint32_t h) { const uint32_t g = seed_group(h); return role ? 2 * g + (uint32_t)strand : g; };
+  auto sub_of = [&](uint32_t h) { return seed_sub(seed_group(h), role, (uint32_t)strand); };
   for (int32_t t = threadIdx.x; t < LIST_CHUNK; t += LIST_BLOCK) {
     uint32_t h; int32_t p;
     if (kmer_of(idx0 + t, h, p)) atomicAdd(&s_cnt[sub_of(h)], 1u);
@@ -70,22 +74,60 @@
   }
 }
 
-__global__ __launch_bounds__(64) void anim_list_scan_kernel(uint32_t* __restrict__ cnt, uint32_t* __restrict__ goff, uint32_t n) {
-  const uint32_t lane = threadIdx.x;
-  uint32_t run = 0, mx = 0;
-  for (uint32_t base = 0; base < n; base += 64) {
-    const uint32_t c = cnt[base + lane];
-    cnt[base + lane] = 0;
-    uint32_t incl = c;
-#pragma unroll
-    for (int o = 1; o < 64; o <<= 1) { const uint32_t t = __shfl_up(incl, o, 64); if ((int)lane >= o) incl += t; }
-    goff[base + lane] = run + incl - c;
-    run += __shfl(incl, 63, 64);
-    mx = c > mx ? c : mx;
-  }
-#pragma unroll
-  for (int o = 32; o > 0; o >>= 1) { const uint32_t t = __shfl_xor(mx, o, 64); mx = t > mx ? t : mx; }
-  if (lane == 0) { goff[n] = run; goff[n + 1] = mx; }
+constexpr int LIST_SCAN_BLOCK = 1024;
+template <int PER>
+__global__ __launch_bounds__(LIST_SCAN_BLOCK) void anim_list_scan_kernel(uint32_t* __restrict__ cnt, uint32_t* __restrict__ goff) {
+  static_assert(PER % SEED_SUB == 0 && PER % 4 == 0, "a thread owns whole coarse groups");
+  constexpr uint32_t n = PER * LIST_SCAN_BLOCK;
+  __shared__ uint32_t s_sum[LIST_SCAN_BLOCK / 64], s_mx[LIST_SCAN_BLOCK / 64], s_cmx[LIST_SCAN_BLOCK / 64];
+  const uint32_t tid = threadIdx.x, lane = tid & 63u, wave = tid >> 6;
+  uint4* const c4 = reinterpret_cast<uint4*>(cnt + tid * PER);
+  uint32_t c[PER];
+#pragma unroll
+  for (int i = 0; i < PER / 4; ++i) {
+    const uint4 v = c4[i];
+    c[4 * i] = v.x; c[4 * i + 1] = v.y; c[4 * i + 2] = v.z; c[4 * i + 3] = v.w;
+    c4[i] = make_uint4(0, 0, 0, 0);
+  }
+  uint32_t sum = 0, mx = 0, cmx = 0;
+#pragma unroll
+  for (int i = 0; i < PER; i += SEED_SUB) {
+    uint32_t run8 = 0;
+#pragma unroll
+    for (int j = 0; j < SEED_SUB; ++j) { run8 += c[i + j]; mx = c[i + j] > mx ? c[i + j] : mx; }
+    sum += run8;
+    cmx = run8 > cmx ? run8 : cmx;
+  }
+  uint32_t incl = sum;
+#pragma unroll
+  for (int o = 1; o < 64; o <<= 1) { const uint32_t t = __shfl_up(incl, o, 64); if ((int)lane >= o) incl += t; }
+#pragma unroll
+  for (int o = 32; o > 0; o >>= 1) {
+    uint32_t t = __shfl_xor(mx, o, 64); mx = t > mx ? t : mx;
+    t = __shfl_xor(cmx, o, 64); cmx = t > cmx ? t : cmx;
+  }
+  if (lane == 63) s_sum[wave] = incl;
+  if (lane == 0) { s_mx[wave] = mx; s_cmx[wave] = cmx; }
+  __syncthreads();
+  uint32_t run = incl - sum;
+  for (uint32_t w = 0; w < wave; ++w) run += s_sum[w];
+  uint4* const g4 = reinterpret_cast<uint4*>(goff + tid * PER);
+#pragma unroll
+  for (int i = 0; i < PER / 4; ++i) {
+    uint4 v;
+    v.x = run; run += c[4 * i];
+    v.y = run; run += c[4 * i + 1];
+    v.z = run; run += c[4 * i + 2];
+    v.w = run; run += c[4 * i + 3];
+    g4[i] = v;
+  }
+  if (tid == LIST_SCAN_BLOCK - 1) {
+    goff[n] = run;
+    uint32_t m = 0, cm = 0;
+    for (uint32_t w = 0; w < LIST_SCAN_BLOCK / 64; ++w) { m = s_mx[w] > m ? s_mx[w] : m; cm = s_cmx[w] > cm ? s_cmx[w] : cm; }
+    goff[n + 1] = m;
+    goff[n + 2] = cm;
+  }
 }
 
 struct SeedRef {
@@ -101,9 +143,9 @@
 __global__ __launch_bounds__(256) void anim_slice_kernel(const SeedQry* __restrict__ sqry, uint32_t n_pairs, SeedSlice* __restrict__ slice) {
   const uint32_t p = blockIdx.x;
   const uint32_t* goff = sqry[p].goff;
-  for (uint32_t g = threadIdx.x; g < SEED_GROUPS; g += 256) {
+  for (uint32_t g = threadIdx.x; g < SEED_CGROUPS; g += 256) {
     if (!goff) { slice[(size_t)g * n_pairs + p] = SeedSlice{0, 0, 0}; continue; }
-    const uint32_t o0 = goff[2 * g], o1 = goff[2 * g + 1], o2 = goff[2 * g + 2];
+    const uint32_t o0 = goff[2 * SEED_SUB * g], o1 = goff[2 * SEED_SUB * g + SEED_SUB], o2 = goff[2 * SEED_SUB * (g + 1)];
     slice[(size_t)g * n_pairs + p] = SeedSlice{o0, o1 - o0, o2 - o1};
   }
 }
@@ -144,11 +186,54 @@
 constexpr int SEED_BLOCK = 1024, SEED_UNROLL = 4;
 constexpr uint32_t SEED_STAGE = 48;
 constexpr size_t SEED_STAGE_BYTES = (SEED_BLOCK / 64) * (SEED_STAGE * sizeof(Match) + 4);
-__global__ __launch_bounds__(SEED_BLOCK) void anim_seed_kernel(const RefDesc* __restrict__ refs, const UnitDesc* __restrict__ units,
-                                                               const SeedRef* __restrict__ srefs, const SeedQry* __restrict__ sqry,
-                                                               const SeedSlice* __restrict__ slice, uint32_t n_pairs,
-                                                               uint32_t slot_mask, Match* __restrict__ buf, uint32_t cap,
-                                                               uint32_t* __restrict__ total, uint32_t* __restrict__ hit_count, int32_t step) {
+__device__ __forceinline__ void seed_stage_hit(Match* stage, uint32_t* stage_n, uint32_t wave, const Match& m, Match* __restrict__ buf,
+                                               uint32_t cap, uint32_t* __restrict__ total, uint32_t* __restrict__ hit_count) {
+  const uint32_t at = atomicAdd(&stage_n[wave], 1u);
+  if (at < SEED_STAGE) {
+    stage[wave * SEED_STAGE + at] = m;
+  } else {
+    const uint32_t ga = atomicAdd(total, 1u);
+    atomicAdd(&hit_count[(uint32_t)m.strand], 1u);
+    if (ga < cap) buf[ga] = m;
+  }
+}
+__device__ __forceinline__ void seed_stage_flush(Match* stage, uint32_t* stage_n, uint32_t wave, uint32_t lane, bool last,
+                                                 Match* __restrict__ buf, uint32_t cap, uint32_t* __restrict__ total,
+                                                 uint32_t* __restrict__ hit_count) {
+  __builtin_amdgcn_wave_barrier();
+  uint32_t n_st = stage_n[wave];
+  if (n_st > SEED_STAGE) n_st = SEED_STAGE;
+  if (n_st >= SEED_STAGE / 2 || (n_st && last)) {
+    static_assert(SEED_STAGE <= 64, "one staged hit per lane at flush time");
+    uint32_t base = 0;
+    if (lane == 0) {
+      base = atomicAdd(total, n_st);
+      stage_n[wave] = 0;
+    }
+    base = __shfl(base, 0);
+    int32_t mr = 0, mq = 0, ml = 0, mu = -1;
+    if (lane < n_st) {
+      const Match& st = stage[wave * SEED_STAGE + lane];
+      mr = st.r; mq = st.q; ml = st.len; mu = st.strand;
+    }
+    const int32_t prev_unit = __shfl_up(mu, 1, 64);
+    const bool start = lane < n_st && (lane == 0 || prev_unit != mu);
+    const uint64_t starts = __ballot(start);
+    if (start) {
+      const uint64_t later = starts >> 1 >> lane;
+      const uint32_t run = later ? (uint32_t)__ffsll((unsigned long long)later) : n_st - lane;
+      atomicAdd(&hit_count[(uint32_t)mu], run);
+    }
+    if (lane < n_st && base + lane < cap) buf[base + lane] = Match{mr, mq, ml, mu};
+    __builtin_amdgcn_wave_barrier();
+  }
+}
+
+__global__ __launch_bounds__(SEED_BLOCK) void anim_seed_pair_kernel(const SeedRef* __restrict__ srefs, const SeedQry* __restrict__ sqry,
+                                                                    const SeedSlice* __restrict__ slice, uint32_t n_pairs,
+                                                                    uint32_t slot_mask, Match* __restrict__ buf, uint32_t cap,
+                                                                    uint32_t* __restrict__ total, uint32_t* __restrict__ hit_count,
+                                                                    int32_t step) {
   extern __shared__ __attribute__((aligned(16))) unsigned long long tab[];
   Match* stage = reinterpret_cast<Match*>(tab + slot_mask + 1);
   uint32_t* stage_n = reinterpret_cast<uint32_t*>(stage + (SEED_BLOCK / 64) * SEED_STAGE);
@@ -158,7 +243,7 @@
   for (uint32_t i = tid; i <= slot_mask; i += SEED_BLOCK) tab[i] = SLOT_EMPTY;
   if (tid < SEED_BLOCK / 64) stage_n[tid] = 0;
   __syncthreads();
-  for (uint32_t e = SR.goff[g] + tid; e < SR.goff[g + 1]; e += SEED_BLOCK) {
+  for (uint32_t e = SR.goff[SEED_SUB * g] + tid; e < SR.goff[SEED_SUB * (g + 1)]; e += SEED_BLOCK) {
     const unsigned long long v = SR.list[e];
     uint32_t slot = (uint32_t)(v >> (SEED_KEY_SHIFT + 5)) & slot_mask;
     while (atomicCAS(&tab[slot], SLOT_EMPTY, v) != SLOT_EMPTY) slot = (slot + 1) & slot_mask;
@@ -205,7 +290,7 @@
         qv[t] = e < c.e_end ? __builtin_nontemporal_load(&c.list[e]) : SLOT_EMPTY;
       }
     };
-    auto process = [&](const Blk& c, const unsigned long long (&qv)[SEED_UNROLL], bool last) {
+    auto process = [&](const Blk& c, const unsigned long long (&qv)[SEED_UNROLL]) {
       const uint32_t unit = 2 * (chunk + c.j) + c.strand;
 #pragma unroll
       for (int t = 0; t < SEED_UNROLL; ++t) {
@@ -229,46 +314,13 @@
               left = diff ? (__ffs(diff) - 1) >> 1 : SEED_STEP;
               report = left < step;
             }
-            if (report) {
-              const Match m{(int32_t)(uint32_t)v, q, left, (int32_t)unit};
-              const uint32_t at = atomicAdd(&stage_n[wave], 1u);
-              if (at < SEED_STAGE) {
-                stage[wave * SEED_STAGE + at] = m;
-              } else {
-                const uint32_t ga = atomicAdd(total, 1u);
-                atomicAdd(&hit_count[unit], 1u);
-                if (ga < cap) buf[ga] = m;
-              }
-            }
+            if (report) seed_stage_hit(stage, stage_n, wave, Match{(int32_t)(uint32_t)v, q, left, (int32_t)unit}, buf, cap, total, hit_count);
           }
           slot_b = (slot_b + 8u) & byte_mask;
           v = *reinterpret_cast<const unsigned long long*>(tab_b + slot_b);
         }
       }
-      __builtin_amdgcn_wave_barrier();
-      uint32_t n_st = stage_n[wave];
-      if (n_st > SEED_STAGE) n_st = SEED_STAGE;
-      if (n_st >= SEED_STAGE / 2 || (n_st && last)) {
-        static_assert(SEED_STAGE <= 64, "one staged hit per lane at flush time");
-        uint32_t base = 0;
-        if (lane == 0) {
-          base = atomicAdd(total, n_st);
-          stage_n[wave] = 0;
-        }
-        base = __shfl(base, 0);
-        Match m{0, 0, 0, -1};
-        if (lane < n_st) m = stage[wave * SEED_STAGE + lane];
-        const int32_t prev_unit = __shfl_up(m.strand, 1, 64);
-        const bool start = lane < n_st && (lane == 0 || prev_unit != m.strand);
-        const uint64_t starts = __ballot(start);
-        if (start) {
-          const uint64_t later = starts >> 1 >> lane;
-          const uint32_t run = later ? (uint32_t)__ffsll((unsigned long long)later) : n_st - lane;
-          atomicAdd(&hit_count[(uint32_t)m.strand], run);
-        }
-        if (lane < n_st && base + lane < cap) buf[base + lane] = m;
-        __builtin_amdgcn_wave_barrier();
-      }
+      seed_stage_flush(stage, stage_n, wave, lane, false, buf, cap, total, hit_count);
     };
     unsigned long long qa[SEED_UNROLL], qb[SEED_UNROLL];
     Blk A = first_from(0, 0);
@@ -276,13 +328,171 @@
     while (A.valid) {
       Blk B = next_of(A);
       if (B.valid) load(B, qb);
-      process(A, qa, !B.valid && chunk + 64 >= my_end);
+      process(A, qa);
       if (!B.valid) break;
       A = next_of(B);
       if (A.valid) load(A, qa);
-      process(B, qb, !A.valid && chunk + 64 >= my_end);
-    }
-  }
+      process(B, qb);
+    }
+  }
+  seed_stage_flush(stage, stage_n, wave, lane, true, buf, cap, total, hit_count);
+}
+
+__device__ __forceinline__ int32_t seed_block_unit(const int32_t* __restrict__ ptab, uint32_t n_qry, uint32_t code) {
+  const int32_t pair = ptab[(size_t)((code >> 1) & 31u) * n_qry + (code >> 6)];
+  return pair >= 0 ? 2 * pair + (int32_t)(code & 1u) : -1;
+}
+
+constexpr int SEED_BLOCK_SLOTS = 32;
+constexpr int SEED_TAB_KEY_SHIFT = 46, SEED_TAB_CTX_SHIFT = 35, SEED_TAB_SLOT_SHIFT = 30;
+constexpr uint32_t SEED_TAB_POS_MASK = (1u << SEED_TAB_SLOT_SHIFT) - 1u, SEED_KEY_MASK = (1u << (32 - SEED_GROUP_BITS)) - 1u;
+static_assert(32 - SEED_GROUP_BITS + 11 + 5 + SEED_TAB_SLOT_SHIFT == 64 && (1 << 5) == SEED_BLOCK_SLOTS, "table entry bit budget");
+struct SeedSlot { const uint64_t* list; const uint32_t* goff; };
+struct SeedBlk {
+  uint32_t slot_begin, slot_end;
+  uint32_t qry_begin, qry_end;
+  uint32_t pair_tab;
+};
+__global__ __launch_bounds__(SEED_BLOCK) void anim_seed_kernel(const SeedBlk* __restrict__ blks, const SeedSlot* __restrict__ slots,
+                                                               const SeedQry* __restrict__ bqry, const int32_t* __restrict__ pair_of,
+                                                               uint32_t slot_mask, uint32_t slot_shift, Match* __restrict__ buf,
+                                                               uint32_t cap, uint32_t* __restrict__ total, uint32_t* __restrict__ hit_count,
+                                                               int32_t step) {
+  extern __shared__ __attribute__((aligned(16))) unsigned long long tab[];
+  Match* stage = reinterpret_cast<Match*>(tab + slot_mask + 1);
+  uint32_t* stage_n = reinterpret_cast<uint32_t*>(stage + (SEED_BLOCK / 64) * SEED_STAGE);
+  const uint32_t g = blockIdx.y;
+  const SeedBlk B = blks[blockIdx.x];
+  const uint32_t tid = threadIdx.x, lane = tid & 63u, wave = tid >> 6;
+  for (uint32_t i = tid; i <= slot_mask; i += SEED_BLOCK) tab[i] = SLOT_EMPTY;
+  if (tid < SEED_BLOCK / 64) stage_n[tid] = 0;
+  __syncthreads();
+  for (uint32_t k = wave; k < B.slot_end - B.slot_begin; k += SEED_BLOCK / 64) {
+    const SeedSlot S = slots[B.slot_begin + k];
+    const uint32_t e_end = S.goff[g + 1];
+    for (uint32_t e = S.goff[g] + lane; e < e_end; e += 64) {
+      const unsigned long long v = S.list[e];
+      const unsigned long long t = (((v >> SEED_KEY_SHIFT) & SEED_KEY_MASK) << SEED_TAB_KEY_SHIFT) | (((v >> 32) & 0x7FFull) << SEED_TAB_CTX_SHIFT) |
+                                   ((unsigned long long)k << SEED_TAB_SLOT_SHIFT) | (uint32_t)v;
+      uint32_t slot = (uint32_t)(t >> (SEED_TAB_KEY_SHIFT + slot_shift)) & slot_mask;
+      while (atomicCAS(&tab[slot], SLOT_EMPTY, t) != SLOT_EMPTY) slot = (slot + 1) & slot_mask;
+    }
+  }
+  __syncthreads();
+  const uint32_t n_qry = B.qry_end - B.qry_begin;
+  const int32_t* __restrict__ ptab = pair_of + B.pair_tab;
+  const uint32_t per_wave = (n_qry + SEED_BLOCK / 64 - 1) / (SEED_BLOCK / 64);
+  const uint32_t my_begin = wave * per_wave;
+  const uint32_t my_end = my_begin + per_wave < n_qry ? my_begin + per_wave : n_qry;
+  const uint32_t sub0 = seed_sub(g, 1, 0), sub1 = seed_sub(g, 1, 1);
+  for (uint32_t chunk = my_begin; chunk < my_end; chunk += 32) {
+    uint32_t n = 0;
+    unsigned long long base = 0;
+    if (chunk + (lane >> 1) < my_end) {
+      const SeedQry Q = bqry[B.qry_begin + chunk + (lane >> 1)];
+      const uint32_t sub = (lane & 1u) ? sub1 : sub0;
+      const uint32_t b = Q.goff[sub];
+      n = Q.goff[sub + 1] - b;
+      base = (unsigned long long)(Q.list + b);
+    }
+    const uint64_t ne = __ballot(n != 0);
+    const uint32_t n_ne = (uint32_t)__popcll(ne);
+    uint32_t src = 0;
+    {
+      uint64_t m = ne;
+      uint32_t lo = 0;
+#pragma unroll
+      for (uint32_t w = 32; w > 0; w >>= 1) {
+        const uint64_t low = w == 64 ? m : (m & ((1ull << w) - 1ull));
+        const uint32_t c = (uint32_t)__popcll(low);
+        if (lane >= lo + c) { lo += c; m >>= w; src += w; } else { m = low; }
+      }
+    }
+    const uint32_t pulled = (uint32_t)__shfl(n, (int)src, 64);
+    const uint32_t cn = lane < n_ne ? pulled : 0u;
+    const unsigned long long cbase = ((unsigned long long)(uint32_t)__shfl((int)(uint32_t)(base >> 32), (int)src, 64) << 32) |
+                                     (uint32_t)__shfl((int)(uint32_t)base, (int)src, 64);
+    uint32_t c = cn;
+#pragma unroll
+    for (int o = 1; o < 64; o <<= 1) { const uint32_t t = __shfl_up(c, o, 64); if ((int)lane >= o) c += t; }
+    const uint32_t T = (uint32_t)__shfl((int)c, 63, 64);
+    c -= cn;
+    const unsigned long long cstart = cbase - (unsigned long long)c * 8ull;
+    auto load = [&](uint32_t E, unsigned long long (&qv)[SEED_UNROLL], uint32_t (&sid)[SEED_UNROLL]) {
+#pragma unroll
+      for (int t = 0; t < SEED_UNROLL; ++t) {
+        const uint32_t R = E + 64u * (uint32_t)t;
+        qv[t] = SLOT_EMPTY;
+        sid[t] = 0;
+        if (R < T) {
+          const uint32_t before = (uint32_t)__popcll(__ballot(lane < n_ne && c < R));
+          uint64_t in_row = __ballot(lane < n_ne && c >= R && c < R + 64u), S = 0;
+          while (in_row) {
+            const int i = __ffsll((unsigned long long)in_row) - 1;
+            S |= 1ull << ((uint32_t)__builtin_amdgcn_readlane((int)c, i) - R);
+            in_row &= in_row - 1ull;
+          }
+          const uint32_t at = before + __builtin_amdgcn_mbcnt_hi((uint32_t)(S >> 32), __builtin_amdgcn_mbcnt_lo((uint32_t)S, 0u)) +
+                              (uint32_t)((S >> lane) & 1ull);
+          const int j = (int)at - 1;
+          const unsigned long long st = ((unsigned long long)(uint32_t)__shfl((int)(uint32_t)(cstart >> 32), j, 64) << 32) |
+                                        (uint32_t)__shfl((int)(uint32_t)cstart, j, 64);
+          sid[t] = (uint32_t)__shfl((int)src, j, 64);
+          if (R + lane < T) qv[t] = __builtin_nontemporal_load(reinterpret_cast<const uint64_t*>(st + 8ull * (R + lane)));
+        }
+      }
+    };
+    auto process = [&](const unsigned long long (&qv)[SEED_UNROLL], const uint32_t (&sid)[SEED_UNROLL]) {
+#pragma unroll
+      for (int t = 0; t < SEED_UNROLL; ++t) {
+        if (qv[t] == SLOT_EMPTY) continue;
+        const uint32_t qhi = (uint32_t)(qv[t] >> 32);
+        const uint32_t qkey = (qhi >> (SEED_KEY_SHIFT - 32)) & SEED_KEY_MASK;
+        const uint32_t qctx = qhi & 0x7FFu;
+        const int32_t q = (int32_t)(uint32_t)qv[t];
+        const uint32_t qcode = ((chunk + (sid[t] >> 1)) << 6) | (sid[t] & 1u);
+        uint32_t slot_b = ((qkey >> slot_shift) & slot_mask) << 3;
+        const uint32_t byte_mask = (slot_mask << 3) | 7u;
+        const char* const tab_b = reinterpret_cast<const char*>(tab);
+        unsigned long long v = *reinterpret_cast<const unsigned long long*>(tab_b + slot_b);
+        while ((uint32_t)v != 0xFFFFFFFFu) {
+          const uint32_t vhi = (uint32_t)(v >> 32);
+          if ((vhi >> (SEED_TAB_KEY_SHIFT - 32)) == qkey) {
+            int32_t left = -1;
+            bool report = true;
+            const uint32_t rctx = (vhi >> (SEED_TAB_CTX_SHIFT - 32)) & 0x7FFu;
+            if (rctx & qctx & 1u) {
+              const uint32_t x = (rctx ^ qctx) >> 1;
+              const uint32_t diff = (x | (x >> 1)) & 0x155u;
+              left = diff ? (__ffs(diff) - 1) >> 1 : SEED_STEP;
+              report = left < step;
+            }
+            if (report) {
+              const uint32_t code = qcode | ((vhi & 7u) << 3) | (((uint32_t)v >> (SEED_TAB_SLOT_SHIFT - 1)) & 6u);
+              const int32_t unit = seed_block_unit(ptab, n_qry, code);
+              if (unit >= 0)
+                seed_stage_hit(stage, stage_n, wave, Match{(int32_t)((uint32_t)v & SEED_TAB_POS_MASK), q, left, unit}, buf, cap, total, hit_count);
+            }
+          }
+          slot_b = (slot_b + 8u) & byte_mask;
+          v = *reinterpret_cast<const unsigned long long*>(tab_b + slot_b);
+        }
+      }
+      seed_stage_flush(stage, stage_n, wave, lane, false, buf, cap, total, hit_count);
+    };
+    unsigned long long qa[SEED_UNROLL], qb[SEED_UNROLL];
+    uint32_t sa[SEED_UNROLL], sb[SEED_UNROLL];
+    constexpr uint32_t STEP = 64u * SEED_UNROLL;
+    if (T) load(0, qa, sa);
+    for (uint32_t E = 0; E < T; E += 2 * STEP) {
+      if (E + STEP < T) load(E + STEP, qb, sb);
+      process(qa, sa);
+      if (E + STEP >= T) break;
+      if (E + 2 * STEP < T) load(E + 2 * STEP, qa, sa);
+      process(qb, sb);
+    }
+  }
+  seed_stage_flush(stage, stage_n, wave, lane, true, buf, cap, total, hit_count);
 }
 
 __global__ __launch_bounds__(1024) void anim_hoff_kernel(const uint32_t* __restrict__ cnt, uint32_t n, uint32_t* __restrict__ hoff,
```
